# Ignaciagothe/tda-eeg-audio

Hardware: AMD Instinct MI355X
Metric: windows/sec end-to-end (dist->Rips H0/H1->Wasserstein), 47-ch EEG (higher is better)
Workload: dtype f64; 1 GPU; configs[4]+configs[2]: 1416 recordings x 5 bands x 15 selected windows = 106200 (EEG 47x250 f64, audio 250 f64) window pairs per pass, the whole job; per pair corr->dist->Rips H0/H1 (EEG 47 pts), tau per recording-band, Takens dim 3 sub 2 + Rips (audio, 23..123 pts over the bands), Wasserstein H0+H1, features, per-recording reductions; one all-gather of the (1416, 5x48) rows per pass; windows_per_pass=106200, windows_per_gpu_per_pass=106200, input_bytes_per_gpu=10195200000, batches_per_pass=1, windows_per_batch=106200, parallelism=recordings dealt over 1 rank(s), one all-gather per pass, batches_in_flight=3, hip_graph=True, batches_rerun_with_full_ladder=0

## Files before the change

### tda_eeg_audio_amd/csrc/corr_dist_dev.h

```cpp
#pragma once
#include "common.h"

#ifndef CD_TCH
#define CD_TCH 32
#define CD_TSH 5
#endif
#define CD_MAXCH 64

typedef double d4 __attribute__((ext_vector_type(4)));



template <int NPRE>
__device__ __forceinline__ void cd_fetch(double (&pre)[NPRE], const double* __restrict__ X, int ld, int n_ch, int c0,
                                         int tc, int tid)
{
    constexpr int CPK = 256 / CD_TCH;
    const int t = tid & (CD_TCH - 1), ch0 = tid >> CD_TSH;
    const int toff = ch0 * ld + t;
    const bool live = t < tc;
#pragma unroll
    for (int k = 0; k < NPRE; ++k) {
        const double* rowk = X + (size_t)(CPK * k) * (size_t)ld + c0;
        pre[k] = (live && ch0 + CPK * k < n_ch) ? rowk[toff] : 0.0;
    }
}
template <int NPRE, int CSP>
__device__ __forceinline__ void cd_stash(const double (&pre)[NPRE], double* tile, const double* mean, int n_ch, int tc,
                                         int tid, bool centre)
{
    double m[NPRE];
#pragma unroll
    for (int k = 0; k < NPRE; ++k) m[k] = centre ? mean[(tid + 256 * k) >> CD_TSH] : 0.0;
    const int t = tid & (CD_TCH - 1);
    const bool live = t < tc;
#pragma unroll
    for (int k = 0; k < NPRE; ++k) {
        const int ch = (tid + 256 * k) >> CD_TSH;
        tile[t * CSP + ch] = live ? pre[k] - m[k] : 0.0;
    }
}

#define CD_RES_CHUNKS (256 / CD_TCH)


template <int NB>
struct CdLayout {
    static constexpr int CP = 16 * NB;
    static constexpr int CSP = CP + 1;
    static constexpr int NBLK = NB * (NB + 1) / 2;
    static constexpr int TILE = CD_TCH * CSP;
    static constexpr int ACCS = NBLK * 256;
    static constexpr size_t BYTES = sizeof(double) * ((size_t)TILE + ACCS + 2 * CP);
    __device__ static __forceinline__ int acc_index(int i, int j)
    {
        const int lo = i < j ? i : j, hi = i < j ? j : i;
        const int r = lo >> 4, s = hi >> 4;
        const int b = r * NB - ((r * (r - 1)) >> 1) + (s - r);
        return (b * 4 + ((lo & 15) >> 2)) * 64 + ((lo & 3) << 4) + (hi & 15);
    }
};

template <int NB, bool RES>
__device__ __forceinline__ void cd_window_products(unsigned char* smem, const double* __restrict__ X, int n_ch, int n_t,
                                                   int ld)
{
    constexpr int CP = 16 * NB;
    constexpr int CSP = CP + 1;
    constexpr int NPRE = CP * CD_TCH / 256;
    constexpr int NBLK = NB * (NB + 1) / 2;
    constexpr int MAXQ = (NBLK + 3) / 4;
    constexpr int NBUF = RES ? CD_RES_CHUNKS : 1;
    double* tile = reinterpret_cast<double*>(smem);
    double* accs = tile + CD_TCH * CSP;
    double* mean = accs + NBLK * 256;
    double* sdev = mean + CP;
    const int tid = threadIdx.x, l = tid & 63, wv = uni(tid >> 6);
    const int n_chunks = (n_t + CD_TCH - 1) / CD_TCH;
    double pre[NBUF][NPRE];
    auto chunk_len = [&](int c) { const int r = n_t - c * CD_TCH; return r < CD_TCH ? r : CD_TCH; };
    const double* lane_base = tile + (l >> 4) * CSP + (l & 15);

    d4 sacc = (d4){0.0, 0.0, 0.0, 0.0};
    auto sum_tile = [&](int tc) {
        if (wv < NB) {
            const double* p0 = lane_base + 16 * wv;
            const int ntr = (tc + 15) >> 4;
            double a[2][2];
            a[0][0] = p0[0]; a[0][1] = p0[4 * CSP];
            for (int d = 0; d < ntr; ++d) {
                const double* p1 = p0 + (16 * d + 8) * CSP;
                a[1][0] = p1[0]; a[1][1] = p1[4 * CSP];
                sacc = __builtin_amdgcn_mfma_f64_16x16x4f64(a[0][0], 1.0, sacc, 0, 0, 0);
                sacc = __builtin_amdgcn_mfma_f64_16x16x4f64(a[0][1], 1.0, sacc, 0, 0, 0);
                const double* p2 = p0 + (16 * d + 16 < CD_TCH ? 16 * d + 16 : 0) * CSP;
                a[0][0] = p2[0]; a[0][1] = p2[4 * CSP];
                sacc = __builtin_amdgcn_mfma_f64_16x16x4f64(a[1][0], 1.0, sacc, 0, 0, 0);
                sacc = __builtin_amdgcn_mfma_f64_16x16x4f64(a[1][1], 1.0, sacc, 0, 0, 0);
            }
            }
    };
    if constexpr (RES) {
#pragma unroll
        for (int c = 0; c < NBUF; ++c)
            if (c < n_chunks) cd_fetch<NPRE>(pre[c], X, ld, n_ch, c * CD_TCH, chunk_len(c), tid);
#pragma unroll
        for (int c = 0; c < NBUF; ++c)
            if (c < n_chunks) {
                cd_stash<NPRE, CSP>(pre[c], tile, mean, n_ch, chunk_len(c), tid, false);
                __syncthreads();
                sum_tile(chunk_len(c));
                __syncthreads();
            }
    } else {
        cd_fetch<NPRE>(pre[0], X, ld, n_ch, 0, chunk_len(0), tid);
        for (int c = 0; c < n_chunks; ++c) {
            cd_stash<NPRE, CSP>(pre[0], tile, mean, n_ch, chunk_len(c), tid, false);
            __syncthreads();
            const int c1 = (c + 1 < n_chunks) ? c + 1 : 0;
            cd_fetch<NPRE>(pre[0], X, ld, n_ch, c1 * CD_TCH, chunk_len(c1), tid);
            sum_tile(chunk_len(c));
            __syncthreads();
        }
    }
    if (wv < NB && (l & 15) == 0) {
#pragma unroll
        for (int v = 0; v < 4; ++v) {
            const int ch = 16 * wv + 4 * v + (l >> 4);
            mean[ch] = ch < n_ch ? sacc[v] / (double)n_t : 0.0;
        }
    }
    __syncthreads();

    auto mfma_tile = [&](int c, int tc) {
        int br[MAXQ], bs[MAXQ], bb[MAXQ];
        d4 acc[MAXQ];
        const int b0 = (wv + 4 * NBLK - ((c * NBLK) & 3)) & 3;
#pragma unroll
        for (int q = 0; q < MAXQ; ++q) {
            int b = b0 + 4 * q, r = 0;
            bb[q] = b;
            if (b >= NBLK) b = 0;
            while (b >= NB - r) { b -= NB - r; ++r; }
            br[q] = r; bs[q] = r + b;
            if (bb[q] < NBLK && c > 0) {
#pragma unroll
                for (int v = 0; v < 4; ++v) acc[q][v] = accs[(bb[q] * 4 + v) * 64 + l];
            } else acc[q] = (d4){0.0, 0.0, 0.0, 0.0};
        }
        double oa[2][MAXQ][2], ob[2][MAXQ][2];
        auto load_ops = [&](int trip, int s) {
#pragma unroll
            for (int q = 0; q < MAXQ; ++q)
                if (bb[q] < NBLK) {
#pragma unroll
                    for (int u = 0; u < 2; ++u) {
                        const double* p = lane_base + (8 * trip + 4 * u) * CSP;
                        oa[s][q][u] = p[16 * br[q]];
                        ob[s][q][u] = p[16 * bs[q]];
                    }
                }
        };
        auto run_ops = [&](int s) {
#pragma unroll
            for (int u = 0; u < 2; ++u)
#pragma unroll
                for (int q = 0; q < MAXQ; ++q)
                    if (bb[q] < NBLK) acc[q] = __builtin_amdgcn_mfma_f64_16x16x4f64(oa[s][q][u], ob[s][q][u], acc[q], 0, 0, 0);
        };
        const int ntr = (tc + 15) >> 4;
        load_ops(0, 0);
        for (int d = 0; d < ntr; ++d) {
            load_ops(2 * d + 1, 1);
            run_ops(0);
            load_ops(2 * d + 2 < CD_TCH / 8 ? 2 * d + 2 : 0, 0);
            run_ops(1);
        }
#pragma unroll
        for (int q = 0; q < MAXQ; ++q)
            if (bb[q] < NBLK) {
#pragma unroll
                for (int v = 0; v < 4; ++v) accs[(bb[q] * 4 + v) * 64 + l] = acc[q][v];
            }
    };
    if constexpr (RES) {
#pragma unroll
        for (int c = 0; c < NBUF; ++c)
            if (c < n_chunks) {
                cd_stash<NPRE, CSP>(pre[c], tile, mean, n_ch, chunk_len(c), tid, true);
                __syncthreads();
                mfma_tile(c, chunk_len(c));
                __syncthreads();
            }
    } else {
        for (int c = 0; c < n_chunks; ++c) {
            cd_stash<NPRE, CSP>(pre[0], tile, mean, n_ch, chunk_len(c), tid, true);
            __syncthreads();
            if (c + 1 < n_chunks) cd_fetch<NPRE>(pre[0], X, ld, n_ch, (c + 1) * CD_TCH, chunk_len(c + 1), tid);
            mfma_tile(c, chunk_len(c));
            __syncthreads();
        }
    }

    const double fact = 1.0 / (double)(n_t - 1);
    if (tid < n_ch) sdev[tid] = sqrt(accs[CdLayout<NB>::acc_index(tid, tid)] * fact);
    __syncthreads();
}
```

### tda_eeg_audio_amd/csrc/rips.hip

```cpp
#include "common.h"
#include "corr_dist_dev.h"
#include "rips_ladder.h"
#include "rips_keys_dev.h"
#include <stdlib.h>

static_assert(TDA_RETRY_AUTO == rips_ladder::AUTO && TDA_RETRY_FIRST_PASS == rips_ladder::FIRST_PASS &&
              TDA_RETRY_ONLY == rips_ladder::ONLY && TDA_RETRY_ONE_STEP == rips_ladder::ONE_STEP &&
              TDA_RETRY_LAST_RUNG == rips_ladder::LAST_RUNG, "rips_ladder::plan takes tda_ctx::retry_policy as it is");

#ifndef CLOUD_NB
#define CLOUD_NB 8192
#endif
#ifndef NARROW_NT
#define NARROW_NT 512
#endif
#ifndef NARROW_WAVES
#define NARROW_WAVES 6
#endif
#if defined(TDA_PROFILE) && !defined(TDA_PROFILE_STOPS_ONLY)
#define NARROW_NB (NARROW_NT == 384 ? 1536 : 1024)
#else
#define NARROW_NB (NARROW_NT == 384 ? 1536 : 2048)
#endif
#define NARROW_EMAX 7626
#define NT_MAX 512
#define RANK_NONE 0x7fffu

#ifdef TDA_PROFILE
__device__ unsigned long long g_prof[48];
#ifdef TDA_PROFILE_STOPS_ONLY
#define PROF_BEGIN() do {} while (0)
#define PROF_RESUME() do {} while (0)
#define PROF_MARK(i) do {} while (0)
#define PROF_COUNT(i, v) do {} while (0)
#define PROF_FLUSH() do {} while (0)
#else
__shared__ unsigned long long prof_lds[48];
#define PROF_BEGIN()                                                       \
    if (threadIdx.x < 48) prof_lds[threadIdx.x] = 0ull;                    \
    __syncthreads();                                                       \
    unsigned long long prof_t0 = clock64()
#define PROF_RESUME() unsigned long long prof_t0 = clock64()
#define PROF_MARK(i)                                                       \
    do {                                                                   \
        unsigned long long prof_t1 = clock64();                            \
        if (threadIdx.x == 0) prof_lds[i] += prof_t1 - prof_t0;            \
        prof_t0 = prof_t1;                                                 \
    } while (0)
#define PROF_COUNT(i, v) do { if (threadIdx.x == 0) prof_lds[i] += (unsigned long long)(v); } while (0)
#define PROF_FLUSH()                                                       \
    do {                                                                   \
        __syncthreads();                                                   \
        if (threadIdx.x < 48 && prof_lds[threadIdx.x]) atomicAdd(&g_prof[threadIdx.x], prof_lds[threadIdx.x]); \
    } while (0)
#endif
__device__ int g_stop_after;
extern "C" __attribute__((visibility("default"))) int tda_profile_stop_after(int n)
{
    return hipMemcpyToSymbol(HIP_SYMBOL(g_stop_after), &n, sizeof(int)) != hipSuccess;
}
#define PROF_STOP(n, cleanup) do { if (g_stop_after == (n)) { cleanup; return; } } while (0)
#define PROF_STOPC(n, cleanup) do { if (g_stop_after == (n) + 100 * prof_chunk) { cleanup; return; } } while (0)
extern "C" __attribute__((visibility("default"))) int tda_profile_read(unsigned long long* out, int reset)
{
    if (hipMemcpyFromSymbol(out, HIP_SYMBOL(g_prof), sizeof(unsigned long long) * 48) != hipSuccess) return 1;
    if (reset) {
        unsigned long long z[48] = {0};
        if (hipMemcpyToSymbol(HIP_SYMBOL(g_prof), z, sizeof(z)) != hipSuccess) return 1;
    }
    return 0;
}
#else
#define PROF_BEGIN() do {} while (0)
#define PROF_RESUME() do {} while (0)
#define PROF_MARK(i) do {} while (0)
#define PROF_COUNT(i, v) do {} while (0)
#define PROF_FLUSH() do {} while (0)
#define PROF_STOP(n, cleanup) do {} while (0)
#define PROF_STOPC(n, cleanup) do {} while (0)
#endif

#define LDS_ORDER() asm volatile("" ::: "memory")

#define LAUNDER(v) asm volatile("" : "+v"(v))
#define WAVE_SYNC()                                            \
    do {                                                       \
        __builtin_amdgcn_fence(__ATOMIC_ACQ_REL, "workgroup"); \
        __builtin_amdgcn_wave_barrier();                       \
    } while (0)

struct SweepShared {
    u64 alive[8];
    int cov_min[2], status, spare, k1, nk, more;
};

typedef unsigned short pk_u16 __attribute__((ext_vector_type(2)));
typedef short pk_i16 __attribute__((ext_vector_type(2)));

template <int W, typename WT>
struct __attribute__((aligned(sizeof(WT)))) Psi {
    WT w[W];
};
template <int W, typename WT>
__device__ __forceinline__ Psi<W, WT> pxor(Psi<W, WT> a, Psi<W, WT> b)
{
    Psi<W, WT> r;
#pragma unroll
    for (int i = 0; i < W; ++i) r.w[i] = a.w[i] ^ b.w[i];
    return r;
}
template <int W, typename WT>
__device__ __forceinline__ bool pnz(Psi<W, WT> a)
{
    WT o = 0;
#pragma unroll
    for (int i = 0; i < W; ++i) o |= a.w[i];
    return o != 0;
}
template <int W, typename WT>
__device__ __forceinline__ Psi<W, WT> pzero()
{
    Psi<W, WT> r;
#pragma unroll
    for (int i = 0; i < W; ++i) r.w[i] = 0;
    return r;
}

__device__ __forceinline__ double wave_min_f64(double v)
{
#pragma unroll
    for (int off = 32; off > 0; off >>= 1) { const double o = __shfl_xor(v, off, 64); v = o < v ? o : v; }
    return v;
}
__device__ __forceinline__ double wave_max_f64(double v)
{
#pragma unroll
    for (int off = 32; off > 0; off >>= 1) { const double o = __shfl_xor(v, off, 64); v = o > v ? o : v; }
    return v;
}

#ifndef TDA_NO_EDGE_TABLE
struct EdgeTable {
    u16 v[8192 + 512];
    constexpr EdgeTable() : v()
    {
        int a = 1, b = 0;
        for (int e = 0; e < 8192 + 512; ++e) { v[e] = (u16)((a << 8) | b); if (++b == a) { ++a; b = 0; } }
    }
};
__device__ const EdgeTable g_edge_ab = EdgeTable();
__device__ __forceinline__ u32 edge_ab(int e) { return (u32)g_edge_ab.v[e]; }
#else
__device__ __forceinline__ u32 edge_ab(int e) { const int a = edge_row(e); return (u32)((a << 8) | (e - tri2(a))); }
#endif

struct WgVote {
    u32* slots;
    int parity;
};
template <int NT>
__device__ __forceinline__ bool wg_any(WgVote& v, bool p)
{
    static_assert(NT % 64 == 0 && NT <= 512, "slots are read as one or two 16-byte words; slots beyond NT / 64 hold zero");
    const bool w = __ballot(p) != 0ull;
    u32* s = v.slots + 8 * v.parity;
    if ((threadIdx.x & 63) == 0) s[threadIdx.x >> 6] = w ? 1u : 0u;
    __syncthreads();
    v.parity ^= 1;
    const uint4 x = *reinterpret_cast<const uint4*>(s);
    u32 r = x.x | x.y | x.z | x.w;
    if (NT > 256) { const uint4 y = *reinterpret_cast<const uint4*>(s + 4); r |= y.x | y.y | y.z | y.w; }
    return r != 0u;
}
template <int NT>
__device__ __forceinline__ bool wg_all(WgVote& v, bool p) { return !wg_any<NT>(v, !p); }

__device__ __forceinline__ int wave_incl_scan_i32(int v)
{
#define TDA_DPP_ADD_(CTRL, RM) v += __builtin_amdgcn_update_dpp(0, v, CTRL, RM, 0xF, true)
    TDA_DPP_ADD_(0x111, 0xF);
    TDA_DPP_ADD_(0x112, 0xF);
    TDA_DPP_ADD_(0x114, 0xF);
    TDA_DPP_ADD_(0x118, 0xF);
    TDA_DPP_ADD_(0x142, 0xA);
    TDA_DPP_ADD_(0x143, 0xC);
#undef TDA_DPP_ADD_
    return v;
}

__device__ __forceinline__ u32 wave_shr1_u32(u32 v) { return (u32)__builtin_amdgcn_update_dpp(0, (int)v, 0x138, 0xF, 0xF, true); }

template <int W, typename WT>
__device__ __forceinline__ Psi<W, WT> last_nonzero_of_owner(Psi<W, WT> y, u32 own1)
{
    constexpr int H = (int)sizeof(WT) / 4;
    u32 x[W * H];
    {
        const bool mine = wave_shr1_u32(own1) == own1;
#pragma unroll
        for (int i = 0; i < W * H; ++i) {
            const u32 below = wave_shr1_u32((u32)((u64)y.w[i / H] >> (32 * (i % H))));
            x[i] = mine ? below : 0u;
        }
    }
#define TDA_STEP_(CTRL)                                                                                              \
    {                                                                                                                \
        u32 any = 0u;                                                                                                \
        _Pragma("unroll") for (int i = 0; i < W * H; ++i) any |= x[i];                                               \
        const bool take = any == 0u && (u32)__builtin_amdgcn_update_dpp(0, (int)own1, CTRL, 0xF, 0xF, true) == own1; \
        _Pragma("unroll") for (int i = 0; i < W * H; ++i) {                                                          \
            const u32 o = (u32)__builtin_amdgcn_update_dpp(0, (int)x[i], CTRL, 0xF, 0xF, true);                      \
            x[i] = take ? o : x[i];                                                                                  \
        }                                                                                                            \
    }
    TDA_STEP_(0x111) TDA_STEP_(0x112) TDA_STEP_(0x114)
#undef TDA_STEP_
    Psi<W, WT> r;
#pragma unroll
    for (int c = 0; c < W; ++c) {
        if constexpr (H == 2) r.w[c] = (WT)(((u64)x[2 * c + 1] << 32) | x[2 * c]);
        else r.w[c] = (WT)x[c];
    }
    return r;
}

__device__ __forceinline__ int edge_flat(u32 pk) { return tri2((int)(pk >> 8)) + (int)(pk & 255u); }

struct Bucketer {
    float dmin, scale, top;
    __device__ __forceinline__ int operator()(u32 key) const
    {
        const float x = fminf((sortable_f32(key) - dmin) * scale, top);
        const int b = (int)x;
        return b < 0 ? 0 : b;
    }
};

template <int NT>
__device__ __forceinline__ void effective_threshold(int n, u32 tkey, const u32* vmax, u32 kmin_thread, u32* red, u32& teff_out, u32& kmin_out)
{
    const int tid = threadIdx.x;
    const int lane = tid & 63;
    const u32 m0 = lane < n ? vmax[lane] : 0xffffffffu, m1 = lane + 64 < n ? vmax[lane + 64] : 0xffffffffu;
    const u32 renc = wave_min_u32_dpp(m0 < m1 ? m0 : m1);
    teff_out = renc < tkey ? renc : tkey;
    if (tid == 0) red[1] = 0xffffffffu;
    __syncthreads();
    const u32 kmin = wave_min_u32_dpp(kmin_thread);
    if (lane == 63) atomicMin(&red[1], kmin);
    __syncthreads();
    kmin_out = red[1];
}

template <int NT, int NB, bool WANT_KEYS>
__device__ __forceinline__ int rank_edges(const u32* key32, int E, u32 teff, u32 kmin, u16* members, u32* cursor, int* wsum, u16* rank,
                          u16* ord, u32* skey)
{
    static_assert(NB % (2 * NT) == 0, "every thread scans whole words");
    constexpr int WPT = NB / NT / 2;
    const int tid = threadIdx.x, lane = tid & 63, wave = tid >> 6;
    Bucketer bk;
    bk.dmin = sortable_f32(kmin);
    bk.top = (float)(NB - 1);
    bk.scale = bk.top / (sortable_f32(teff) - bk.dmin);
    for (int i = tid; i < NB / 2; i += NT) cursor[i] = 0u;
    __syncthreads();
#pragma unroll 4
    for (int e = tid; e < E; e += NT) {
        const u32 k = key32[e];
        u32 b = 0xffffu;
        if (k <= teff) { b = (u32)bk(k); atomicAdd(&cursor[b >> 1], 1u << (16 * (b & 1))); }
        rank[e] = (u16)b;
    }
    __syncthreads();
    {
        u32 w[WPT];
        int s = 0;
#pragma unroll
        for (int i = 0; i < WPT; ++i) {
            const u32 x = cursor[tid * WPT + i];
            const int c0 = (int)(x & 0xffffu), c1 = (int)(x >> 16);
            w[i] = (u32)s | ((u32)(s + c0) << 16);
            s += c0 + c1;
        }
        const int incl = wave_incl_scan_i32(s);
        if (lane == 63) wsum[wave] = incl;
        __syncthreads();
        int basep = incl - s;
        for (int q = 0; q < wave; ++q) basep += wsum[q];
        const u32 add = (u32)basep * 0x00010001u;
#pragma unroll
        for (int i = 0; i < WPT; ++i) cursor[tid * WPT + i] = w[i] + add;
    }
    __syncthreads();
#pragma unroll 4
    for (int e = tid; e < E; e += NT) {
        const u32 b = rank[e];
        if (b != 0xffffu) {
            const int sh = 16 * (int)(b & 1u);
            const u32 old = atomicAdd(&cursor[b >> 1], 1u << sh);
            members[(old >> sh) & 0xffffu] = (u16)e;
        }
    }
    __syncthreads();
    const u16* cur16 = reinterpret_cast<const u16*>(cursor);
    const int Ev = uni((int)cur16[NB - 1]);
#pragma unroll 4
    for (int e = tid; e < E; e += NT) {
        const u32 b = rank[e];
        u32 r = RANK_NONE;
        if (b != 0xffffu) {
            const u32 k = key32[e];
            const int lo = b ? (int)cur16[b - 1] : 0, hi = (int)cur16[b];
            int c = 0;
            for (int j = lo; j < hi; ++j) {
                const u32 m = members[j];
                const u32 km = key32[m];
                c += (km < k || (km == k && m < (u32)e)) ? 1 : 0;
            }
            r = (u32)(lo + c);
        }
        rank[e] = (u16)r;
    }
    __syncthreads();
#pragma unroll 4
    for (int e = tid; e < E; e += NT) {
        const u32 r = rank[e];
        if (r != RANK_NONE) {
            ord[r] = (u16)edge_ab(e);
            if (WANT_KEYS) skey[r] = key32[e];
        }
    }
    __syncthreads();
    return Ev;
}

#if defined(TDA_PROFILE) && !defined(TDA_PROFILE_STOPS_ONLY)
#define NARROW_LDS ((160 * 1024 / 3 / 1280) * 1280 - 384)
#else
#define NARROW_LDS ((160 * 1024 / 3 / 1280) * 1280)
#endif
#define NARROW_PMAX 124
#define NARROW_DIM 3
#ifdef TDA_DEBUG_PTS
#define NL_GUARD 16
#else
#define NL_GUARD 0
#endif
#define NL_A16(x) (((x) + 15) & ~15)
struct NL {
    static constexpr int E = NARROW_EMAX;
    static constexpr int RANK = 0;
    static constexpr int PSI = NL_A16(2 * E) + NL_GUARD;
    static constexpr int MEMBERS = NL_A16(4 * (E + 4));
    static constexpr int CURSOR = NL_A16(MEMBERS + 2 * E);
    static constexpr int RSCR = CURSOR + 2 * NARROW_NB;
    static constexpr int TOTAL = NARROW_LDS;
    static constexpr int AUX = TOTAL - NL_GUARD - NL_A16(NARROW_PMAX * NARROW_DIM * 8);
    static constexpr int MISC = AUX - NL_GUARD - NL_A16(8752 + 8 * 32);
    static constexpr int REGION = MISC - NL_GUARD - PSI;
    static_assert(RSCR + 720 <= AUX - NL_GUARD, "the ranking arrays must end in front of the points");
    static_assert(MEMBERS >= 4 * (E + 4) && CURSOR >= MEMBERS + 2 * E, "room for the walk's padding: skey[E .. E + 3] (rank_edges_narrow)");
    static_assert(E < 0x8000 && RANK_NONE >= E, "rank and flat index of a slot share a register (rank_edges_narrow)");
    static_assert(REGION >= 2 * E + 8 * 512, "the first chunks must fit: class vectors of 2 NT ranks next to the whole of ord");
};

template <int NT, int NB>
__device__ __forceinline__ int rank_edges_narrow(u32* skey, int E, u32 teff, u32 kmin, u16* sidx, u32* cursor, int* wsum,
                                                 u16* rank, u16* ord)
{
    static_assert(NB % (2 * NT) == 0, "every thread scans whole words");
    constexpr int WPT = NB / NT / 2;
    constexpr int EPT = (NARROW_EMAX + NT - 1) / NT;
    static_assert(EPT <= 32, "one bit per edge of the thread");
    const int tid = threadIdx.x, lane = tid & 63, wave = tid >> 6;
    Bucketer bk;
    bk.dmin = sortable_f32(kmin);
    bk.top = (float)(NB - 1);
    bk.scale = bk.top / (sortable_f32(teff) - bk.dmin);
    for (int i = tid; i < NB / 2; i += NT) cursor[i] = 0u;
    __syncthreads();
    u32 kreg[EPT], breg[EPT];
    u32 beyond = 0u;
#pragma unroll
    for (int i = 0; i < EPT; ++i) {
        const int e = tid + i * NT;
        breg[i] = 0xffffffffu;
        if (e < E) {
            const u32 k = skey[e];
            kreg[i] = k;
            if (k <= teff) { const u32 b = (u32)bk(k); breg[i] = b; atomicAdd(&cursor[b >> 1], 1u << (16 * (b & 1))); }
            else beyond |= 1u << i;
        }
    }
    __syncthreads();
    {
        u32 w[WPT];
        int s = 0;
#pragma unroll
        for (int i = 0; i < WPT; ++i) {
            const u32 x = cursor[tid * WPT + i];
            const int c0 = (int)(x & 0xffffu), c1 = (int)(x >> 16);
            w[i] = (u32)s | ((u32)(s + c0) << 16);
            s += c0 + c1;
        }
        const int incl = wave_incl_scan_i32(s);
        if (lane == 63) wsum[wave] = incl;
        __syncthreads();
        int basep = incl - s;
        for (int q = 0; q < wave; ++q) basep += wsum[q];
        const u32 add = (u32)basep * 0x00010001u;
#pragma unroll
        for (int i = 0; i < WPT; ++i) cursor[tid * WPT + i] = w[i] + add;
        if (tid == NT - 1) {
            const int total = basep + s;
            skey[total] = 0xffffffffu; skey[total + 1] = 0xffffffffu; skey[total + 2] = 0xffffffffu; skey[total + 3] = 0xffffffffu;
        }
    }
    __syncthreads();
#pragma unroll
    for (int i = 0; i < EPT; ++i) {
        const u32 b = breg[i];
        if (b != 0xffffffffu) {
            const int sh = 16 * (int)(b & 1u);
            const u32 slot = (atomicAdd(&cursor[b >> 1], 1u << sh) >> sh) & 0xffffu;
            skey[slot] = kreg[i];
            sidx[slot] = (u16)(tid + i * NT);
        }
    }
    __syncthreads();
    const u16* cur16 = reinterpret_cast<const u16*>(cursor);
    const int Ev = uni((int)cur16[NB - 1]);
    u32 re[EPT];
#pragma unroll
    for (int i = 0; i < EPT; ++i) {
        const int s = tid + i * NT;
        re[i] = 0xffffffffu;
        if (s < Ev) {
            const u32 k = skey[s];
            const u32 e = (u32)sidx[s];
            const u32 b = (u32)bk(k);
            const int lo = b ? (int)cur16[b - 1] : 0, hi = (int)cur16[b];
            int c = 0;
            u32 q = 4u * (u32)lo;
            const u32 q_hi = 4u * (u32)hi, q_end = 4u * (u32)Ev;
            u64 once = 0ull, twice = 0ull;
#pragma unroll 1
            do {
                const u32* p = reinterpret_cast<const u32*>(reinterpret_cast<const unsigned char*>(skey) + min(q, q_end));
                u32 km[4];
#pragma unroll
                for (int t = 0; t < 4; ++t) km[t] = p[t];
#pragma unroll
                for (int t = 0; t < 4; ++t) {
                    c += km[t] < k ? 1 : 0;
                    const u64 m = __ballot(km[t] == k);
                    twice |= once & m;
                    once |= m;
                }
                q += 16u;
            } while (__any(q < q_hi));
            if ((twice >> lane) & 1ull) {
                c = 0;
#pragma unroll 1
                for (int j = lo; j < hi; ++j) {
                    const u32 km = skey[j];
                    c += (km < k || (km == k && (u32)sidx[j] < e)) ? 1 : 0;
                }
            }
            re[i] = ((u32)(lo + c) << 16) | e;
        }
    }
    __syncthreads();
#pragma unroll
    for (int i = 0; i < EPT; ++i) {
        if (re[i] != 0xffffffffu) {
            const u32 r = re[i] >> 16, e = re[i] & 0xffffu;
            rank[e] = (u16)r;
            ord[r] = (u16)edge_ab((int)e);
        }
        if (beyond & (1u << i)) rank[tid + i * NT] = (u16)RANK_NONE;
    }
    __syncthreads();
    return Ev;
}

struct RipsOut {
    double* h0; int h0_cap; int* h0_cnt;
    double* h1; int h1_cap; int* h1_cnt;
    int* status;
    int* retry_list = nullptr;
};

struct RipsLayout {
    int off_members;
    int off_rank, off_ord, off_aux, off_misc;
    int total;
    int off_psi, psi_bytes, off_cursor, off_rscr;
    int guard[5], n_guard;
};

#define TDA_WIN_LDS_GUARD 0x100
#ifndef TDA_SOLO_PRIO
#define TDA_SOLO_PRIO 3
#endif
#define TDA_SOLO_BEGIN() __builtin_amdgcn_s_setprio(TDA_SOLO_PRIO)
#define TDA_SOLO_END() __builtin_amdgcn_s_setprio(0)

#define TDA_POLL_LIMIT (1 << 16)
#ifndef TDA_TURN_SLEEP
#define TDA_TURN_SLEEP 4
#endif
#ifdef TDA_DEBUG_PTS
__device__ int g_fault;
extern "C" __attribute__((visibility("default"))) int tda_debug_inject(int what)
{
    return hipMemcpyToSymbol(HIP_SYMBOL(g_fault), &what, sizeof(int)) != hipSuccess;
}
#define TDA_FAULT(n) (g_fault == (n))
#else
#define TDA_FAULT(n) false
#endif
#ifdef TDA_DEBUG_PTS
#define GUARD_BYTES 16
__device__ __forceinline__ void guard_write(unsigned char* smem, const RipsLayout& L)
{
    if ((int)threadIdx.x < 4 * L.n_guard) reinterpret_cast<u32*>(smem + L.guard[threadIdx.x >> 2] - GUARD_BYTES)[threadIdx.x & 3] = 0xC0FFEE00u + threadIdx.x;
    __syncthreads();
}
__device__ __forceinline__ int guard_check(unsigned char* smem, const RipsLayout& L)
{
    __syncthreads();
    bool bad = false;
    if ((int)threadIdx.x < 4 * L.n_guard) bad = reinterpret_cast<u32*>(smem + L.guard[threadIdx.x >> 2] - GUARD_BYTES)[threadIdx.x & 3] != 0xC0FFEE00u + threadIdx.x;
    return __syncthreads_or(bad ? 1 : 0) ? TDA_WIN_LDS_GUARD : 0;
}
#else
#define GUARD_BYTES 0
__device__ __forceinline__ void guard_write(unsigned char*, const RipsLayout&) {}
__device__ __forceinline__ int guard_check(unsigned char*, const RipsLayout&) { return 0; }
#endif

#define MISC_COMP 0
#define MISC_CAND 512
#define MISC_WV (512 + 128)
#define MISC_MIN (512 + 192)
#define MISC_DONE (512 + 208)
#define MISC_SORTCNT (512 + 224)
#define MISC_SHARED (MISC_DONE + NT_MAX)
#define MISC_CKEY (MISC_SHARED + 96)
#define MISC_LIST MISC_CKEY
#define MISC_LIST_BYTES (4 * NT_MAX + 1280)
#define MISC_ADJ (MISC_LIST + MISC_LIST_BYTES)
#define MISC_ADJC (MISC_ADJ + 128 * 16)
#define MISC_BRANK (MISC_ADJC + 128 * 16)
#define MISC_BYTES(ncls) (MISC_BRANK + 8 * (ncls))

template <int NT, int NVW, int W, typename WT, bool NARROW, class KEYFN>
__device__ __forceinline__ void rips_sweep(int n, int E, int Ev, const u16* rank, const u16* ord, Psi<W, WT>* psi, int psi_bytes,
                           unsigned char* misc, KEYFN keyfn, double* h0, int h0_cap, double* h1, int h1_cap,
                           int& out_k0, int& out_k1, int& out_status)
{
    static_assert(!NARROW || W == 1, "the narrow layout is the point-cloud first pass");
    int psi_cap = 0;
    const int tid0 = threadIdx.x;
    const int lane0 = tid0 & 63, wave = uni(tid0 >> 6);
    int* brank = reinterpret_cast<int*>(misc + MISC_BRANK);
    u64* cand = reinterpret_cast<u64*>(misc + MISC_CAND);
    unsigned char* done = misc + MISC_DONE;
    SweepShared* shared = reinterpret_cast<SweepShared*>(misc + MISC_SHARED);
    u64* adj = reinterpret_cast<u64*>(misc + MISC_ADJ);
    constexpr int WB = 8 * (int)sizeof(WT);
    float* bkey = reinterpret_cast<float*>(misc + MISC_BRANK + 4 * WB * W);
    u64* adjc = reinterpret_cast<u64*>(misc + MISC_ADJC);
    int* tcum = reinterpret_cast<int*>(misc + MISC_COMP + 256);
    int* ecum = reinterpret_cast<int*>(misc + MISC_COMP + 320);
    int eset = 0;

    if constexpr (!NARROW) for (int e = tid0; e < E; e += NT) psi[e] = pzero<W, WT>();
    for (int i = tid0; i < WB * W; i += NT) { brank[i] = -1; bkey[i] = 0.f; }
    for (int i = tid0; i < 256; i += NT) { adj[i] = 0ull; adjc[i] = 0ull; }
    if (tid0 == 0) {
        u32* lc = reinterpret_cast<u32*>(misc + MISC_MIN);
        lc[0] = 0u; lc[1] = 0xffffffffu; lc[2] = 0u;
        lc[3] = 0u;
        shared->status = 0;
    }
    if (tid0 < 16) {
        reinterpret_cast<u32*>(misc + MISC_WV)[tid0] = 0u;
        cand[tid0] = 0ull;
    }
    __syncthreads();

    WgVote vote{reinterpret_cast<u32*>(misc + MISC_WV), 0};
    WT alive[W];
#pragma unroll
    for (int c = 0; c < W; ++c) alive[c] = 0;
    int k0 = 0, k1 = 0, merges = 0, status = 0;
    int compA = lane0, compB = lane0 + 64;

    int clen = NT;
    int ordcls = 0;
    int cov_next = tid0;
#ifdef TDA_PROFILE
    int prof_rneed = 0, prof_chunk = -1;
#endif
    PROF_RESUME();
    for (int r0 = 0; r0 < Ev && !status; r0 += clen) {
        int tid = tid0;
        LAUNDER(tid);
        const int lane = tid & 63;
        clen = NT;
        PROF_MARK(15);
#ifdef TDA_PROFILE
        ++prof_chunk;
#endif
        PROF_COUNT(23, 1);
        const int r = r0 + tid;
        const bool valid = r < Ev;
        int a = 1, b = 0;
        if (valid) { const u32 pk = ord[r]; a = (int)(pk >> 8); b = (int)(pk & 255u); }
        const int tab = tri2(a) + b;
        const int slot = NARROW ? r : tab;
        if constexpr (NARROW) {
            psi_cap = (psi_bytes - 2 * (E - r0)) >> 2;
            if (r < psi_cap) psi[r] = pzero<W, WT>();
        }
        u64 M[NVW], M0[NVW];
        u64 Aj[NVW], Bj[NVW];
#pragma unroll
        for (int w = 0; w < NVW; ++w) { M[w] = 0; M0[w] = 0; Aj[w] = 0; Bj[w] = 0; }
        if (valid) {
#pragma unroll
            for (int w = 0; w < NVW; ++w) { Aj[w] = adj[2 * a + w]; Bj[w] = adj[2 * b + w]; M0[w] = Aj[w] & Bj[w]; }
        }
        {
            volatile u32* turn = reinterpret_cast<volatile u32*>(misc + MISC_MIN) + 2;
            if (wave > 0) {
                int trips = 0;
                for (;;) {
                    const u32 t = (u32)uni((int)*turn);
                    if (t >= (u32)wave) break;
                    if (++trips > TDA_POLL_LIMIT) { if (lane == 0) turn[1] = 1u; break; }
                    if (t + 1u < (u32)wave) __builtin_amdgcn_s_sleep(TDA_TURN_SLEEP); else __builtin_amdgcn_s_sleep(0);
                }
            }
            __builtin_amdgcn_fence(__ATOMIC_ACQUIRE, "workgroup");
            if (valid) {
#pragma unroll
                for (int w = 0; w < NVW; ++w) M[w] = (Aj[w] | adjc[2 * a + w]) & (Bj[w] | adjc[2 * b + w]);
                atomicOr(reinterpret_cast<unsigned long long*>(&adjc[2 * a + (b >> 6)]), 1ull << (b & 63));
                atomicOr(reinterpret_cast<unsigned long long*>(&adjc[2 * b + (a >> 6)]), 1ull << (a & 63));
            }
            LDS_ORDER();
            if (lane == 0 && !(TDA_FAULT(1) && wave == 3)) *turn = (u32)wave + 1u;
        }
        if (valid) {
            const int ta0 = tri2(a), tb0 = tri2(b);
#pragma unroll
            for (int w = 0; w < NVW; ++w) {
                u64 cc = (Aj[w] | adjc[2 * a + w]) & (Bj[w] | adjc[2 * b + w]) & ~M[w];
                while (cc) {
                    const int v0 = 64 * w + __builtin_ctzll(cc); cc &= cc - 1ull;
                    const bool ok1 = cc != 0ull; const int v1 = ok1 ? 64 * w + __builtin_ctzll(cc) : v0; cc &= cc - 1ull;
                    const int t0 = tri2(v0), t1 = tri2(v1);
                    const u32 xa0 = rank[v0 < a ? ta0 + v0 : t0 + a], xb0 = rank[v0 < b ? tb0 + v0 : t0 + b];
                    const u32 xa1 = rank[v1 < a ? ta0 + v1 : t1 + a], xb1 = rank[v1 < b ? tb0 + v1 : t1 + b];
                    if ((int)(xa0 > xb0 ? xa0 : xb0) < r) M[w] |= 1ull << (v0 & 63);
                    if (ok1 && (int)(xa1 > xb1 ? xa1 : xb1) < r) M[w] |= 1ull << (v1 & 63);
                }
            }
        }
        u64 many = 0;
#pragma unroll
        for (int w = 0; w < NVW; ++w) many |= M[w];
        const bool is_cand = valid && many == 0;
        int vstar = 0, d1 = 0, d2 = 0, q1 = 0, q2 = 0;
        {
            u64 many0 = 0;
#pragma unroll
            for (int w = 0; w < NVW; ++w) many0 |= M0[w];
            if (many0) {
                if (NVW == 1 || M0[0]) vstar = __builtin_ctzll(M0[0]);
                else vstar = 64 + __builtin_ctzll(M0[NVW - 1]);
            } else if (many) {
                if (NVW == 1 || M[0]) vstar = __builtin_ctzll(M[0]);
                else vstar = 64 + __builtin_ctzll(M[NVW - 1]);
            }
            if (valid && many != 0) {
                d1 = pair_index(a, vstar); d2 = pair_index(b, vstar);
                q1 = (int)rank[d1] - r0; q2 = (int)rank[d2] - r0;
                if (TDA_FAULT(2) && tid == 77 && q1 >= 0) q1 = tid;
            }
        }
        PROF_MARK(4);
        PROF_STOPC(11, out_k0 = k0; out_k1 = k1; out_status = 0);
        u64* mbal = reinterpret_cast<u64*>(misc + MISC_COMP);
        u64* zbal = mbal + 8;
        int* offs = reinterpret_cast<int*>(mbal + 16);
        u16* freebits = reinterpret_cast<u16*>(misc + MISC_CKEY);
        float mykey = 0.f;
        if (is_cand) mykey = keyfn(r, a, b);
        {
            const u64 bal = __ballot(is_cand), zb = __ballot(is_cand && mykey == 0.0f);
            if (lane == 0) { cand[wave] = bal; zbal[wave] = zb; }
        }
        done[tid] = 0;
        if (tid < 9) tcum[tid] = 0;
        __syncthreads();
        PROF_MARK(21);
        PROF_STOPC(12, out_k0 = k0; out_k1 = k1; out_status = 0);
        int nfree = 0;
#pragma unroll
        for (int c = 0; c < W; ++c) nfree += __builtin_popcountll((u64)(WT)~alive[c]);
        int ncand = 0;
#pragma unroll
        for (int w = 0; w < NT / 64; ++w) ncand += __builtin_popcountll(cand[w]);
        int btot = 0;
        if (ncand > 0) {
        const bool par = ncand > 24;
        const int lblA0 = compA, lblB0 = compB;
        int qpar = NT;
        if (par) {
            int* bcomp = reinterpret_cast<int*>(misc + MISC_LIST + 1024);
            u32* bbest2 = reinterpret_cast<u32*>(bcomp + 128);
            int* bpar = reinterpret_cast<int*>(bcomp + 384);
            auto rounds = [&](int limit) {
                if (wave == 0) { bcomp[lane] = lblA0; bcomp[64 + lane] = lblB0; }
                if (tid < 256) bbest2[tid] = 0xffffffffu;
                __syncthreads();
                bool live = is_cand && tid < limit, picked = false;
                for (int round = 0; round < 64; ++round) {
                    u32* bbest = bbest2 + 128 * (round & 1);
                    int ca = 0, cb2 = 0;
                    if (live) {
                        ca = bcomp[a]; cb2 = bcomp[b];
                        if (ca == cb2) live = false;
                        else { atomicMin(&bbest[ca], (u32)tid); atomicMin(&bbest[cb2], (u32)tid); }
                    }
                    if (!wg_any<NT>(vote, live)) break;
                    if (live && (bbest[ca] == (u32)tid || bbest[cb2] == (u32)tid)) { picked = true; live = false; }
                    if (wave == 0) {
                        TDA_SOLO_BEGIN();
                        int pp[2];
#pragma unroll
                        for (int h = 0; h < 2; ++h) {
                            const int me = lane + 64 * h;
                            pp[h] = me;
                            const u32 bp = bbest[me];
                            if (bp != 0xffffffffu) {
                                const u32 pk = ord[r0 + (int)bp];
                                const int oa = bcomp[pk >> 8], ob = bcomp[pk & 255u];
                                pp[h] = oa == me ? ob : oa;
                                if (bbest[pp[h]] == bp && me < pp[h]) pp[h] = me;
                            }
                        }
                        bpar[lane] = pp[0]; bpar[64 + lane] = pp[1];
                        for (int it = 0; it < 8; ++it) {
                            const int p0 = bpar[lane], p1 = bpar[64 + lane];
                            const int g0 = bpar[p0], g1 = bpar[p1];
                            if (__ballot(g0 != p0 || g1 != p1) == 0ull) break;
                            bpar[lane] = g0; bpar[64 + lane] = g1;
                        }
                        const int c0 = bcomp[lane], c1 = bcomp[64 + lane];
                        const int n0 = bpar[c0], n1 = bpar[c1];
                        bcomp[lane] = n0; bcomp[64 + lane] = n1;
                        u32* other = bbest2 + 128 * ((round + 1) & 1);
                        other[lane] = 0xffffffffu; other[64 + lane] = 0xffffffffu;
                        TDA_SOLO_END();
                    }
                    __syncthreads();
                }
                const u64 mb = __ballot(picked);
                if (lane == 0) mbal[wave] = mb;
                __syncthreads();
            };
            rounds(NT);
            int nbirth = 0, wcut = -1, before = 0;
#pragma unroll
            for (int w = 0; w < NT / 64; ++w) {
                const int nb = __builtin_popcountll(cand[w] & ~mbal[w]);
                if (wcut < 0 && nbirth + nb > nfree) { wcut = w; before = nbirth; }
                nbirth += nb;
            }
            if (wcut >= 0) {
                u64 bw = cand[wcut] & ~mbal[wcut];
                for (int k = before; k < nfree; ++k) bw &= bw - 1ull;
                qpar = 64 * wcut + __builtin_ctzll(bw);
                PROF_COUNT(26, 1);
                __syncthreads();
                rounds(qpar);
            }
            if (wave == 0) { compA = bcomp[lane]; compB = bcomp[64 + lane]; }
        }
        if (wave == 0) {
            TDA_SOLO_BEGIN();
            const u64 candv = cand[lane & 7];
            int q = par ? qpar : NT, births = 0;
            const bool walk = !par;
            for (int g = 0; g < NT / 64 && walk; ++g) {
                u64 cb = q == NT ? rl64(candv, g) : 0ull;
                u64 mm = 0ull;
                if (cb) {
                    PROF_COUNT(20, __builtin_popcountll(cb));
                    const u32 pkv = ord[r0 + 64 * g + lane < E ? r0 + 64 * g + lane : E - 1];
                    while (cb) {
                        const int l = __builtin_ctzll(cb);
                        cb &= cb - 1;
                        const u32 pk = rl32(pkv, l);
                        const int qa = (int)(pk >> 8), qb = (int)(pk & 255u);
                        int ca, cbb;
                        if (NVW == 1) {
                            ca = (int)rl32((u32)compA, qa);
                            cbb = (int)rl32((u32)compA, qb);
                        } else {
                            const int a0 = (int)rl32((u32)compA, qa & 63), a1 = (int)rl32((u32)compB, qa & 63);
                            const int b0 = (int)rl32((u32)compA, qb & 63), b1 = (int)rl32((u32)compB, qb & 63);
                            ca = qa < 64 ? a0 : a1;
                            cbb = qb < 64 ? b0 : b1;
                        }
                        const bool same = ca == cbb, open = q == NT;
                        q = (open && same && births == nfree) ? 64 * g + l : q;
                        births += same ? 1 : 0;
                        const int cnew = (q == NT) ? ca : cbb;
                        compA = compA == cbb ? cnew : compA;
                        if (NVW == 2) compB = compB == cbb ? cnew : compB;
                        mm |= (!same && q == NT) ? (1ull << l) : 0ull;
                    }
                }
                if (lane == 0) mbal[g] = mm;
            }
            int nb = 0, nr = 0, nm = 0;
            if (lane < NT / 64) {
                u64 cg = cand[lane];
                if (64 * lane >= q) cg = 0ull;
                else if (q < 64 * lane + 64) cg &= (1ull << (q - 64 * lane)) - 1ull;
                const u64 mg = mbal[lane], zg = zbal[lane];
                nb = __builtin_popcountll(cg & ~mg); nr = __builtin_popcountll(mg & ~zg); nm = __builtin_popcountll(mg);
            }
            int pb = 0, pr = 0, tb = 0, tr = 0, tm = 0;
#pragma unroll
            for (int w = 0; w < NT / 64; ++w) {
                const int xb = (int)rl32((u32)nb, w), xr = (int)rl32((u32)nr, w), xm = (int)rl32((u32)nm, w);
                if (w < lane) { pb += xb; pr += xr; }
                tb += xb; tr += xr; tm += xm;
            }
            if (lane < NT / 64) { offs[lane] = pb; offs[8 + lane] = pr; }
            if (lane == 0) { offs[16] = tb; offs[17] = tr; offs[18] = tm; offs[19] = q; }
            TDA_SOLO_END();
        } else {
            for (int t = tid - 64; t < WB * W; t += NT - 64) {
                const int cw = t / WB, bit = t & (WB - 1);
                int rk = 0;
                bool fr = false;
#pragma unroll
                for (int c = 0; c < W; ++c) {
                    const WT f_ = (WT)~alive[c];
                    if (c < cw) rk += __builtin_popcountll((u64)f_);
                    if (c == cw) { rk += __builtin_popcountll((u64)(f_ & (((WT)1 << bit) - (WT)1))); fr = (f_ >> bit) & (WT)1; }
                }
                if (fr) freebits[rk] = (u16)t;
            }
        }
        __syncthreads();
        PROF_MARK(22);
        PROF_STOPC(13, out_k0 = k0; out_k1 = k1; out_status = 0);
        clen = uni(offs[19]);
        if (clen == 0) status |= TDA_WIN_CLASS_OVERFLOW;
        if (clen < NT) PROF_COUNT(14, 1);
        bool mrg = is_cand && ((mbal[wave] >> lane) & 1ull);
        bool birth = is_cand && !mrg && tid < clen;
        bool row = mrg && mykey != 0.0f;
        const u64 below = (1ull << lane) - 1ull;
        const int bpre = offs[wave] + __builtin_popcountll(__ballot(birth) & below);
        const int rpre = offs[8 + wave] + __builtin_popcountll(__ballot(row) & below);
        btot = uni(offs[16]);
        const int rtot = uni(offs[17]), mtot = uni(offs[18]);
        if (!status) {
            if (row) {
                const int pos = k0 + rpre;
                if (pos < h0_cap) { h0[2 * pos] = 0.0; h0[2 * pos + 1] = (double)mykey; }
            }
            k0 += rtot; merges += mtot;
            if (birth) {
                const int idx = (int)freebits[bpre];
                const int cw = idx / WB, bit = idx & (WB - 1);
                Psi<W, WT> nv = pzero<W, WT>();
#pragma unroll
                for (int c = 0; c < W; ++c)
                    if (c == cw) nv.w[c] = ((WT)1 << bit);
                if (!NARROW || r < psi_cap) psi[slot] = nv;
                brank[idx] = r;
                bkey[idx] = mykey;
            }
            if (W == 1 && wave == 0 && btot > 0) {
                const int nal = __builtin_popcountll((u64)alive[0]);
                if (lane >= nal && lane < nal + btot) ordcls = (int)freebits[lane - nal];
            }
            int left = btot;
#pragma unroll
            for (int c = 0; c < W; ++c) {
                const u64 f_ = (u64)(WT)~alive[c];
                const int pc = __builtin_popcountll(f_);
                if (left >= pc) { alive[c] = (WT)~(WT)0; left -= pc; }
                else if (left > 0) {
                    int lo = 0, hi = 63;
                    while (lo < hi) {
                        const int mid = (lo + hi) >> 1;
                        if (__builtin_popcountll(f_ & ((2ull << mid) - 1ull)) >= left) hi = mid; else lo = mid + 1;
                    }
                    alive[c] |= (WT)(f_ & ((2ull << lo) - 1ull));
                    left = 0;
                }
            }
        }
        }
        if (status) break;
        PROF_MARK(5);
        PROF_STOPC(14, out_k0 = k0; out_k1 = k1; out_status = 0);
        bool quiet = btot == 0;
#pragma unroll
        for (int c = 0; c < W; ++c) quiet = quiet && alive[c] == 0;
        u32* lcnt = reinterpret_cast<u32*>(misc + MISC_MIN);
        if (quiet) PROF_COUNT(24, 1);
#ifdef TDA_PROFILE
        if (!quiet) prof_rneed = r0 + clen;
#endif
        if constexpr (NARROW) {
            if (!quiet && r0 + NT > psi_cap) { status |= TDA_WIN_CLASS_OVERFLOW; break; }
        }
        if (!quiet) {
        const bool apparent = valid && many != 0 && tid < clen;
        bool pending = apparent;
        Psi<W, WT> base = pzero<W, WT>();
        const int s1 = NARROW ? q1 + r0 : d1, s2 = NARROW ? q2 + r0 : d2;
        if (apparent && q1 < 0 && q2 < 0) {
            base = pxor(psi[s1], psi[s2]);
            psi[slot] = base;
            pending = false;
        }
        volatile unsigned char* vdone = done;
        LDS_ORDER();
        if (!pending) vdone[tid] = 1;
#ifdef TDA_PROFILE
#ifndef TDA_PROFILE_STOPS_ONLY
        if (pending) atomicAdd(&prof_lds[33], 1ull);
#endif
        PROF_COUNT(34, 1);
#endif
        int idle_trips = 0;
        while (__ballot(pending)) {
            PROF_COUNT(32, 1);
            bool ready = false;
            if (pending) ready = (q1 < 0 || vdone[q1]) && (q2 < 0 || vdone[q2]);
            const u64 rbal = __ballot(ready);
            __builtin_amdgcn_fence(__ATOMIC_ACQUIRE, "workgroup");
            if (ready) {
                base = pxor(psi[s1], psi[s2]);
                psi[slot] = base;
                LDS_ORDER();
                vdone[tid] = 1;
                pending = false;
            }
            if (!rbal) {
                if (++idle_trips > TDA_POLL_LIMIT) {
                    if (lane == 0) reinterpret_cast<volatile u32*>(misc + MISC_MIN)[3] = 1u;
                    if (pending) vdone[tid] = 1;
                    break;
                }
                __builtin_amdgcn_s_sleep(1);
            }
        }
        __syncthreads();
        PROF_MARK(6);
        PROF_STOPC(15, out_k0 = k0; out_k1 = k1; out_status = 0);
        u32 m0, m1, m2 = 0u, m3 = 0u;
        {
            u64 rem[NVW];
#pragma unroll
            for (int w = 0; w < NVW; ++w) rem[w] = 0ull;
            if (apparent) {
                u64 comp[NVW];
#pragma unroll
                for (int w = 0; w < NVW; ++w) comp[w] = 0ull;
                if (NVW == 1 || vstar < 64) comp[0] = 1ull << vstar;
                else comp[NVW - 1] = 1ull << (vstar - 64);
#pragma unroll
                for (int w = 0; w < NVW; ++w) { comp[w] |= adj[2 * vstar + w] & M[w]; rem[w] = M[w] & ~comp[w]; }
                bool changed = true;
                while (changed) {
                    changed = false;
#pragma unroll
                    for (int w = 0; w < NVW; ++w) {
                        u64 rr = rem[w];
                        while (rr) {
                            int u[4]; bool ok[4];
#pragma unroll
                            for (int k = 0; k < 4; ++k) {
                                ok[k] = rr != 0ull;
                                u[k] = ok[k] ? 64 * w + __builtin_ctzll(rr) : vstar;
                                rr &= rr - 1ull;
                            }
                            u64 nb[4][NVW];
#pragma unroll
                            for (int k = 0; k < 4; ++k)
#pragma unroll
                                for (int x = 0; x < NVW; ++x) nb[k][x] = adj[2 * u[k] + x];
#pragma unroll
                            for (int k = 0; k < 4; ++k) {
                                u64 hit = 0ull;
#pragma unroll
                                for (int x = 0; x < NVW; ++x) hit |= nb[k][x] & comp[x];
                                if (ok[k] && hit) {
                                    comp[w] |= 1ull << (u[k] & 63);
                                    rem[w] &= ~(1ull << (u[k] & 63));
                                    changed = true;
                                }
                            }
                        }
                    }
                    u64 anyr = 0ull;
#pragma unroll
                    for (int w = 0; w < NVW; ++w) anyr |= rem[w];
                    if (!anyr) break;
                }
            }
            m0 = (u32)rem[0]; m1 = (u32)(rem[0] >> 32);
            if (NVW == 2) { m2 = (u32)rem[NVW - 1]; m3 = (u32)(rem[NVW - 1] >> 32); }
        }
        PROF_MARK(16);
        PROF_STOPC(16, out_k0 = k0; out_k1 = k1; out_status = 0);
        constexpr int ES = 4 + W * (int)sizeof(WT);
        constexpr bool SORTED = W == 1;
        constexpr int LMAX = SORTED ? MISC_LIST_BYTES / ES : 256;
        constexpr int LCAP = (MISC_LIST_BYTES / ES) < LMAX ? (MISC_LIST_BYTES / ES) : LMAX;
        constexpr int LPL = (LCAP + 63) / 64;
        static_assert(LCAP * ES <= MISC_LIST_BYTES, "the list stays inside its area");
        constexpr bool FTAB = WB * W * (int)sizeof(Psi<W, WT>) <= MISC_LIST_BYTES;
        constexpr int KMAX = FTAB ? 64 : LCAP;
        unsigned char* list = misc + MISC_LIST;
        u32* tlist = reinterpret_cast<u32*>(adjc);
        static_assert(4 * NT <= 128 * 16 && NT / 64 <= 8, "the work list lives in adjc; nine words per sum");
        const bool cum_lane = lane == 8 || (lane < 8 && lane > wave);
        const int ntri = __builtin_popcount(m0) + __builtin_popcount(m1) + __builtin_popcount(m2) + __builtin_popcount(m3);
        int tstart, ttot;
        const int incl_ = wave_incl_scan_i32(ntri);
        const int wtri = __builtin_amdgcn_readlane(incl_, 63);
        {
            if (wtri != 0 && cum_lane) atomicAdd(&tcum[lane], wtri);
            __syncthreads();
            tstart = tcum[wave] + incl_ - ntri;
            ttot = uni(tcum[8]);
        }
#ifdef TDA_PROFILE
        {
            const int ntri = __builtin_popcount(m0) + __builtin_popcount(m1) + __builtin_popcount(m2) + __builtin_popcount(m3);
#ifndef TDA_PROFILE_STOPS_ONLY
            if (ntri) atomicAdd(&prof_lds[27], (unsigned long long)ntri);
            if (apparent) atomicAdd(&prof_lds[28], 1ull);
            if (ntri) atomicAdd(&prof_lds[29], 1ull);
#endif
        }
#endif
        int list_rounds = 0;
        while (true) {
            u64 left[NVW];
            left[0] = (u64)m0 | ((u64)m1 << 32);
            if (NVW == 2) left[NVW - 1] = (u64)m2 | ((u64)m3 << 32);
            int nxt = tstart;
            int lbase = 0;
#ifdef TDA_PROFILE
            {
                PROF_COUNT(43, (ttot + NT - 1) / NT); PROF_COUNT(44, ttot); PROF_COUNT(47, 1);
#ifndef TDA_PROFILE_STOPS_ONLY
                if (wtri != 0 && lane == 0) atomicAdd(&prof_lds[45], 1ull);
#endif
            }
#endif
            for (int t0 = 0; t0 < ttot; t0 += NT) {
                int* ec = ecum + 16 * eset;
                eset ^= 1;
                if (tid < 9) ec[tid] = 0;
#pragma unroll
                for (int wi = 0; wi < NVW; ++wi) {
                    while (left[wi] != 0ull && (u32)(nxt - t0) < (u32)NT) {
                        const int v = 64 * wi + __builtin_ctzll(left[wi]);
                        left[wi] &= left[wi] - 1ull;
                        tlist[nxt - t0] = ((u32)tid << 8) | (u32)v;
                        ++nxt;
                    }
                }
                __syncthreads();
                u32 code = 0u;
                Psi<W, WT> y = pzero<W, WT>();
                bool keep = false;
                u64 kb = 0ull;
                if (t0 + (wave << 6) < ttot) {
                    const bool item = t0 + tid < ttot;
                    if (item) {
                        code = tlist[tid];
                        const int op = (int)(code >> 8), v = (int)(code & 255u);
                        const u32 pk = ord[r0 + op];
                        const int oa = (int)(pk >> 8), ob = (int)(pk & 255u);
                        const int ta_ = tri2(oa), tb_ = tri2(ob);
                        const int tv = (int)(__umul24((u32)v, (u32)(v - 1)) >> 1);
                        const int fa = v < oa ? ta_ + v : tv + oa;
                        const int fb = v < ob ? tb_ + v : tv + ob;
                        const int ja = NARROW ? (int)rank[fa] : fa;
                        const int jb = NARROW ? (int)rank[fb] : fb;
                        y = pxor(pxor(psi[ja], psi[jb]), psi[NARROW ? r0 + op : ta_ + ob]);
                    }
                    const Psi<W, WT> pv = last_nonzero_of_owner(y, item ? (code >> 8) + 1u : 0u);
                    keep = pnz(y) && pnz(pxor(y, pv));
                    kb = __ballot(keep);
                }
                if (kb != 0ull && cum_lane) atomicAdd(&ec[lane], __builtin_popcountll(kb));
                __syncthreads();
                const int pos = lbase + ec[wave] + (int)__builtin_amdgcn_mbcnt_hi((u32)(kb >> 32), __builtin_amdgcn_mbcnt_lo((u32)kb, 0u));
                lbase += uni(ec[8]);
                if (keep && pos < LCAP) {
                    *reinterpret_cast<u32*>(list + ES * pos) = code;
#pragma unroll
                    for (int c = 0; c < W; ++c)
                        *reinterpret_cast<WT*>(list + ES * pos + 4 + c * (int)sizeof(WT)) = y.w[c];
                }
            }
            if (lbase == 0) {
                PROF_MARK(17);
                PROF_STOPC(17, out_k0 = k0; out_k1 = k1; out_status = 0);
                break;
            }
            __syncthreads();
            PROF_MARK(17);
            PROF_STOPC(17, out_k0 = k0; out_k1 = k1; out_status = 0);
            const u32 cnt = (u32)lbase;
            const bool complete = cnt <= (u32)LCAP;
            PROF_COUNT(11, 1);
            PROF_COUNT(12, cnt);
            if (!complete) PROF_COUNT(13, 1);
            if (cnt > 2u * (u32)LCAP) PROF_COUNT(46, 1);
            WT alive_before[W];
#pragma unroll
            for (int c = 0; c < W; ++c) alive_before[c] = alive[c];
            if (wave == 0) {
                TDA_SOLO_BEGIN();
                const int nl = complete ? (int)cnt : LCAP;
                constexpr int LREG = SORTED ? 1 : LPL;
                u32 ek[LREG];
                Psi<W, WT> ev[LREG];
                auto load_block = [&](int q, u32& k, Psi<W, WT>& x) {
                    const int idx = lane + 64 * q;
                    k = 0xffffffffu; x = pzero<W, WT>();
                    if (idx < nl) {
                        k = *reinterpret_cast<const u32*>(list + ES * idx);
#pragma unroll
                        for (int c = 0; c < W; ++c)
                            x.w[c] = *reinterpret_cast<const WT*>(list + ES * idx + 4 + c * (int)sizeof(WT));
                    }
                };
#pragma unroll
                for (int q = 0; q < LREG; ++q) load_block(q, ek[q], ev[q]);
                const int lb = lane & (WB - 1);
                int brk[W];
                float bky[W];
#pragma unroll
                for (int c = 0; c < W; ++c) {
                    brk[c] = lane < WB ? brank[WB * c + lb] : -1;
                    bky[c] = lane < WB ? bkey[WB * c + lb] : 0.f;
                }
                int nalive0 = W == 1 ? __builtin_popcountll((u64)alive[0]) : 0;
                Psi<W, WT> vimg = pzero<W, WT>();
                u32 mycode = 0u, myrk = 0u;
                float mybirth = 0.f;
                int nk = 0, more = 0;
                const int nq = (nl + 63) >> 6;
                PROF_MARK(30);
                if constexpr (SORTED) {
                    WT kvec = 0;
                    WT cm = lane < nalive0 ? (WT)1 << ordcls : (WT)0;
                    bool stop = false;
                    for (int q = 0; q < nq && !stop; ++q) {
                        WT v = ev[0].w[0];
                        const u32 myk = ek[0];
                        if (q + 1 < nq) load_block(q + 1, ek[0], ev[0]);
                        for (int k = 0; k < nk; ++k) {
                            const WT m = (WT)1 << rl32(mycode, k);
                            const WT w = sizeof(WT) == 8 ? (WT)rl64((u64)kvec, k) : (WT)rl32((u32)kvec, k);
                            if (v & m) v ^= w;
                        }
                        u64 nz = __ballot(v != 0);
                        while (nz) {
                            if (nk == KMAX) { more = 1; stop = true; break; }
                            const int src = __builtin_ctzll(nz);
                            const WT wvw = sizeof(WT) == 8 ? (WT)rl64((u64)v, src) : (WT)rl32((u32)v, src);
                            const u64 ob = __ballot((cm & wvw) != 0);
                            if (!ob) { status |= TDA_WIN_CLASS_OVERFLOW; stop = true; break; }
                            const int opos = 63 - __builtin_clzll(ob);
                            const int ybit = (int)rl32((u32)ordcls, opos);
                            const WT ybm = (WT)1 << ybit;
                            if (v & ybm) v ^= wvw;
                            nz = __ballot(v != 0);
                            const u32 kk = rl32(myk, src);
                            const float ybirth = __uint_as_float(rl32(__float_as_uint(bky[0]), ybit));
                            cm &= (WT)~ybm;
                            const bool me = lane == nk;
                            WT vi = vimg.w[0];
                            if (vi & ybm) vi ^= wvw;
                            vimg.w[0] = me ? (WT)(wvw & (WT)~ybm) : vi;
                            mycode = me ? (u32)ybit : mycode;
                            myrk = me ? (u32)(r0 + (int)((kk >> 8) & 0xffffu)) : myrk;
                            mybirth = me ? ybirth : mybirth;
                            kvec = me ? wvw : kvec;
                            alive[0] &= (WT)~ybm;
                            ++nk;
                        }
                    }
                    if (nk > 0) {
                        const bool keep = cm != 0;
                        const u64 keepb = __ballot(keep);
                        const int below = (int)__builtin_amdgcn_mbcnt_hi((u32)(keepb >> 32), __builtin_amdgcn_mbcnt_lo((u32)keepb, 0u));
                        const int dst = keep ? below : __builtin_popcountll(keepb) + (lane - below);
                        ordcls = __builtin_amdgcn_ds_permute(dst << 2, ordcls);
                    }
                } else
                while (true) {
                    u32 mk = 0xffffffffu;
#pragma unroll
                    for (int q = 0; q < LPL; ++q)
                        if (q < nq && pnz(ev[q]) && ek[q] < mk) mk = ek[q];
                    const u32 best = wave_min_u32_dpp(mk);
                    if (best == 0xffffffffu) break;
                    if (nk == KMAX) { more = 1; break; }
                    const int src = __builtin_ctzll(__ballot(mk == best));
                    Psi<W, WT> mine = pzero<W, WT>();
#pragma unroll
                    for (int q = 0; q < LPL; ++q)
                        if (q < nq && ek[q] == best) mine = ev[q];
                    Psi<W, WT> wv;
#pragma unroll
                    for (int c = 0; c < W; ++c) {
                        if (sizeof(WT) == 8) wv.w[c] = (WT)rl64((u64)mine.w[c], src);
                        else wv.w[c] = (WT)rl32((u32)mine.w[c], src);
                    }
                    const int rk = r0 + (int)(best >> 8);
                    int ybit, ycw;
                    float ybirth;
                    if (W == 1) {
                        const u64 ob = __ballot(lane < nalive0 && (((u64)wv.w[0] >> ordcls) & 1ull));
                        if (!ob) { status |= TDA_WIN_CLASS_OVERFLOW; break; }
                        const int opos = 63 - __builtin_clzll(ob);
                        ybit = (int)rl32((u32)ordcls, opos);
                        ycw = 0;
                        ybirth = __uint_as_float(rl32(__float_as_uint(bky[0]), ybit));
                        const int up = __builtin_amdgcn_update_dpp(0, ordcls, 0x130, 0xF, 0xF, true);
                        if (lane >= opos) ordcls = up;
                        --nalive0;
                    } else {
                        int candv = -1, cwl = 0;
                        float byl = 0.f;
#pragma unroll
                        for (int c = 0; c < W; ++c)
                            if (lane < WB && ((wv.w[c] >> lb) & (WT)1) && brk[c] > candv) { candv = brk[c]; cwl = c; byl = bky[c]; }
                        const int bestr = wave_max_i32_dpp(candv);
                        const u64 ybal = __ballot(candv == bestr && candv >= 0);
                        if (!ybal) { status |= TDA_WIN_CLASS_OVERFLOW; break; }
                        ybit = __builtin_ctzll(ybal);
                        ycw = (int)rl32((u32)cwl, ybit);
                        ybirth = __uint_as_float(rl32(__float_as_uint(byl), ybit));
                    }
                    if (FTAB) {
                        WT sel = 0;
#pragma unroll
                        for (int c = 0; c < W; ++c)
                            if (c == ycw) sel = (vimg.w[c] >> ybit) & (WT)1;
                        if (lane < nk && sel) vimg = pxor(vimg, wv);
                        if (lane == nk) {
                            vimg = wv;
#pragma unroll
                            for (int c = 0; c < W; ++c)
                                if (c == ycw) vimg.w[c] &= (WT)~((WT)1 << ybit);
                            mycode = ((u32)ycw << 8) | (u32)ybit; myrk = (u32)rk; mybirth = ybirth;
                        }
                    } else {
                        const u32 pkk = ord[rk];
                        const float key = keyfn(rk, (int)(pkk >> 8), (int)(pkk & 255u));
                        if (key > ybirth) {
                            if (k1 < h1_cap && lane == 0) { h1[2 * k1] = (double)ybirth; h1[2 * k1 + 1] = (double)key; }
                            ++k1;
                        }
                        if (lane == 0) {
                            *reinterpret_cast<u32*>(list + ES * nk) = ((u32)ycw << 8) | (u32)ybit;
#pragma unroll
                            for (int c = 0; c < W; ++c) *reinterpret_cast<WT*>(list + ES * nk + 4 + c * (int)sizeof(WT)) = wv.w[c];
                        }
                    }
#pragma unroll
                    for (int q = 0; q < LPL; ++q) {
                        if (q >= nq) break;
                        WT sel = 0;
#pragma unroll
                        for (int c = 0; c < W; ++c)
                            if (c == ycw) sel = (ev[q].w[c] >> ybit) & (WT)1;
                        if (sel) ev[q] = pxor(ev[q], wv);
                    }
#pragma unroll
                    for (int c = 0; c < W; ++c)
                        if (c == ycw) alive[c] &= (WT)~((WT)1 << ybit);
                    ++nk;
                }
                PROF_MARK(31);
                PROF_COUNT(10, nk);
                if (FTAB) {
                    const bool mine_ok = lane < nk;
                    float key = 0.f;
                    if (mine_ok) {
                        const u32 pkk = ord[(int)myrk];
                        key = keyfn((int)myrk, (int)(pkk >> 8), (int)(pkk & 255u));
                    }
                    const bool emit = mine_ok && key > mybirth;
                    const u64 bal = __ballot(emit);
                    const int pos = k1 + __builtin_popcountll(bal & ((1ull << lane) - 1ull));
                    if (emit && pos < h1_cap) { h1[2 * pos] = (double)mybirth; h1[2 * pos + 1] = (double)key; }
                    k1 += __builtin_popcountll(bal);
                    if (mine_ok) {
                        Psi<W, WT>* ftab = reinterpret_cast<Psi<W, WT>*>(list);
                        ftab[WB * (int)(mycode >> 8) + (int)(mycode & 255u)] = vimg;
                    }
                }
                if (lane == 0) {
#pragma unroll
                    for (int c = 0; c < W; ++c) shared->alive[c] = (u64)alive[c];
                    shared->k1 = k1; shared->nk = nk; shared->more = more; shared->status = status;
                }
                TDA_SOLO_END();
            }
            __syncthreads();
            PROF_MARK(18);
            PROF_STOPC(18, out_k0 = k0; out_k1 = k1; out_status = 0);
            WT kmask[W];
#pragma unroll
            for (int c = 0; c < W; ++c) {
                const WT na = sizeof(WT) == 8 ? (WT)uni64(shared->alive[c]) : (WT)uni((int)(u32)shared->alive[c]);
                kmask[c] = alive_before[c] & (WT)~na; alive[c] = na;
            }
            k1 = uni(shared->k1);
            const int nk = uni(shared->nk);
            const bool more = uni(shared->more) != 0;
            status = uni(shared->status);
            if (status) break;
            if (FTAB) {
                const Psi<W, WT>* ftab = reinterpret_cast<const Psi<W, WT>*>(list);
                const int seen_end = r0 + clen < Ev ? r0 + clen : Ev;
#pragma unroll 4
                for (int rr = tid; rr < seen_end; rr += NT) {
                    const int e = NARROW ? rr : edge_flat(ord[rr]);
                    const Psi<W, WT> p = psi[e];
                    WT anyh = 0;
#pragma unroll
                    for (int c = 0; c < W; ++c) anyh |= p.w[c] & kmask[c];
                    if (!anyh) continue;
                    Psi<W, WT> q;
#pragma unroll
                    for (int c = 0; c < W; ++c) q.w[c] = p.w[c] & (WT)~kmask[c];
#pragma unroll
                    for (int c = 0; c < W; ++c) {
                        u64 hh = (u64)(p.w[c] & kmask[c]);
                        while (hh) {
                            const int bit = __builtin_ctzll(hh);
                            hh &= hh - 1ull;
                            q = pxor(q, ftab[WB * c + bit]);
                        }
                    }
                    psi[e] = q;
                }
            } else {
                for (int j0 = 0; j0 < nk; j0 += 4) {
                    u32 kc[4];
                    Psi<W, WT> kw[4];
#pragma unroll
                    for (int j = 0; j < 4; ++j) {
                        const int jj = j0 + j < nk ? j0 + j : j0;
                        kc[j] = j0 + j < nk ? *reinterpret_cast<const u32*>(list + ES * jj) : 0xffffffffu;
#pragma unroll
                        for (int c = 0; c < W; ++c) kw[j].w[c] = *reinterpret_cast<const WT*>(list + ES * jj + 4 + c * (int)sizeof(WT));
                    }
#pragma unroll 4
                    for (int rr = tid; rr < (r0 + clen < Ev ? r0 + clen : Ev); rr += NT) {
                        const int e = NARROW ? rr : edge_flat(ord[rr]);
                        Psi<W, WT> p = psi[e];
                        bool changed = false;
#pragma unroll
                        for (int j = 0; j < 4; ++j) {
                            if (kc[j] == 0xffffffffu) continue;
                            const int jcw = (int)(kc[j] >> 8), jbit = (int)(kc[j] & 255u);
                            WT sel = 0;
#pragma unroll
                            for (int c = 0; c < W; ++c)
                                if (c == jcw) sel = (p.w[c] >> jbit) & (WT)1;
                            if (sel) { p = pxor(p, kw[j]); changed = true; }
                        }
                        if (changed) psi[e] = p;
                    }
                }
            }
            PROF_MARK(19);
            PROF_STOPC(19, out_k0 = k0; out_k1 = k1; out_status = 0);
            if (complete && !more) break;
            if (++list_rounds > 4 * NT) { status |= TDA_WIN_CLASS_OVERFLOW; break; }
            __syncthreads();
        }
        }
        if (valid && tid < clen) {
            atomicOr(reinterpret_cast<unsigned long long*>(&adj[2 * a + (b >> 6)]), 1ull << (b & 63));
            atomicOr(reinterpret_cast<unsigned long long*>(&adj[2 * b + (a >> 6)]), 1ull << (a & 63));
        }
        if (tid < 256) adjc[tid] = 0ull;
        if (tid == 0) {
            lcnt[0] = 0u; lcnt[1] = 0xffffffffu; lcnt[2] = 0u; shared->cov_min[0] = 0x7fffffff;
            if (lcnt[3]) shared->status = TDA_WIN_NOT_CONVERGED;
        }
        __syncthreads();
        if (uni(shared->status) & TDA_WIN_NOT_CONVERGED) { status |= TDA_WIN_NOT_CONVERGED; break; }
        bool calm = status == 0 && clen == NT;
#pragma unroll
        for (int c = 0; c < W; ++c) calm = calm && alive[c] == 0;
        if (calm && !quiet) PROF_COUNT(2, 1);
        if (calm) {
            int from = r0 + clen;
            int rr = (NT & (NT - 1)) == 0 ? from + ((tid - from) & (NT - 1)) : from + (((tid - from) % NT) + NT) % NT;
            rr = rr > cov_next ? rr : cov_next;
            int ru;
            for (int round = 0;; ++round) {
                PROF_COUNT(41, 1);
                bool covered = true;
                while (rr < Ev) {
                    const u32 pk = ord[rr];
                    const int ea = (int)(pk >> 8), eb = (int)(pk & 255u);
                    u64 common = adj[2 * ea] & adj[2 * eb];
                    if (NVW == 2) common |= adj[2 * ea + 1] & adj[2 * eb + 1];
                    if (common == 0ull) { covered = false; break; }
                    rr += NT;
                }
                int* cmin = &shared->cov_min[round & 1];
                {
                    const u32 wmin = wave_min_u32_dpp(covered ? 0x7fffffffu : (u32)rr);
                    if (lane == 0 && wmin != 0x7fffffffu) atomicMin(reinterpret_cast<unsigned int*>(cmin), wmin);
                }
                __syncthreads();
                ru = uni(*cmin);
                if (ru >= Ev || ru == from) break;
                if (tid == 0) shared->cov_min[(round + 1) & 1] = 0x7fffffff;
                for (int r2 = from + tid; r2 < ru; r2 += NT) {
                    const u32 pk = ord[r2];
                    const int ea = (int)(pk >> 8), eb = (int)(pk & 255u);
                    atomicOr(reinterpret_cast<unsigned long long*>(&adj[2 * ea + (eb >> 6)]), 1ull << (eb & 63));
                    atomicOr(reinterpret_cast<unsigned long long*>(&adj[2 * eb + (ea >> 6)]), 1ull << (ea & 63));
                }
                PROF_COUNT(35, ru - from);
                from = ru;
                __syncthreads();
                if (round == 31) break;
            }
            cov_next = rr;
            if (ru >= Ev) { PROF_COUNT(25, 1); PROF_MARK(7); break; }
            PROF_COUNT(42, 1);
            if (from > r0 + clen) {
                if constexpr (NARROW) {
                    const int cap = (psi_bytes - 2 * (E - from)) >> 2;
                    for (int r2 = r0 + clen + tid; r2 < (from < cap ? from : cap); r2 += NT) psi[r2] = pzero<W, WT>();
                    __syncthreads();
                }
                clen = from - r0;
            }
        }
        PROF_MARK(7);
        PROF_STOPC(20, out_k0 = k0; out_k1 = k1; out_status = 0);
    }
#ifdef TDA_PROFILE
    PROF_COUNT(36, prof_rneed > 4096 ? 1 : 0); PROF_COUNT(37, prof_rneed > 4608 ? 1 : 0); PROF_COUNT(38, prof_rneed > 5120 ? 1 : 0);
    PROF_COUNT(39, prof_rneed); PROF_COUNT(40, Ev);
#endif
    const int ncomp = n - merges;
    for (int i = 0; i < ncomp; ++i) {
        if (k0 < h0_cap && tid0 == 0) { h0[2 * k0] = 0.0; h0[2 * k0 + 1] = (double)INFINITY; }
        ++k0;
    }
#pragma unroll
    for (int c = 0; c < W; ++c) {
        u64 al = (u64)alive[c];
        while (al) {
            const int bit = __builtin_ctzll(al);
            al &= al - 1;
            if (k1 < h1_cap && tid0 == 0) { h1[2 * k1] = (double)bkey[WB * c + bit]; h1[2 * k1 + 1] = (double)INFINITY; }
            ++k1;
        }
    }
    if (k1 > h1_cap) status |= TDA_WIN_H1_TRUNCATED;
    out_k0 = k0; out_k1 = k1; out_status = status;
}


#define TOT_NW 128
#define TOT_SLOTS 8
#define TOT_SLOT_WORDS ((size_t)8128 * TOT_NW)
#define RETRY_GRID 512
#define RETRY_GRID_WIDE 64

template <int NT, class KEYFN>
__device__ __forceinline__ void rips_sweep_total(int n, int E, int Ev, const u16* rank, const u16* ord, float* bkey, unsigned char* misc,
                                 u64* __restrict__ psi_g, KEYFN keyfn, double* h0, int h0_cap, double* h1, int h1_cap,
                                 int& out_k0, int& out_k1, int& out_status)
{
    constexpr int NWV = NT / 64;
    const int tid = threadIdx.x, lane = tid & 63, wave = uni(tid >> 6);
    u64* adj = reinterpret_cast<u64*>(misc + MISC_ADJ);
    int* comp = reinterpret_cast<int*>(misc + MISC_COMP);
    u32* flags = reinterpret_cast<u32*>(misc + MISC_WV);
    u64* yv = reinterpret_cast<u64*>(misc + MISC_LIST);
    u64* cur = yv + TOT_NW;
    u32* nzbit = reinterpret_cast<u32*>(misc + MISC_ADJ + 4096);
    u32* alivebit = nzbit + 256;
    static_assert(MISC_LIST_BYTES >= 2 * TOT_NW * 8, "scratch of the total sweep");
    for (int i = tid; i < 256; i += NT) { adj[i] = 0ull; nzbit[i] = 0u; alivebit[i] = 0u; }
    for (int v = tid; v < 128; v += NT) comp[v] = v;
    __syncthreads();
    int k0 = 0, k1 = 0, merges = 0, nborn = 0, nalive = 0;
    auto stored = [&](int rr) { return (nzbit[rr >> 5] >> (rr & 31)) & 1u; };
    for (int r = 0; r < Ev; ++r) {
        const u32 pk = (u32)uni((int)ord[r]);
        const int a = (int)(pk >> 8), b = (int)(pk & 255u);
        const u64 M0 = uni64(adj[2 * a] & adj[2 * b]), M1 = uni64(adj[2 * a + 1] & adj[2 * b + 1]);
        if ((M0 | M1) == 0ull) {
            const int ca = uni(comp[a]), cb = uni(comp[b]);
            const float key = keyfn(r, a, b);
            __syncthreads();
            if (ca != cb) {
                for (int v = tid; v < n; v += NT) if (comp[v] == cb) comp[v] = ca;
                if (key != 0.0f) {
                    if (tid == 0 && k0 < h0_cap) { h0[2 * k0] = 0.0; h0[2 * k0 + 1] = (double)key; }
                    ++k0;
                }
                ++merges;
            } else {
                const int c = nborn++;
                if (tid == 0) { bkey[c] = key; nzbit[r >> 5] |= 1u << (r & 31); alivebit[c >> 5] |= 1u << (c & 31); }
                for (int w = tid; w < TOT_NW; w += NT) psi_g[(size_t)r * TOT_NW + w] = (w == (c >> 6)) ? 1ull << (c & 63) : 0ull;
                ++nalive;
            }
        } else if (nalive > 0) {
            const int vstar = M0 ? __builtin_ctzll(M0) : 64 + __builtin_ctzll(M1);
            const int s1 = uni((int)rank[pair_index(a, vstar)]), s2 = uni((int)rank[pair_index(b, vstar)]);
            const bool z1 = !stored(s1), z2 = !stored(s2);
            u64 bw = 0ull;
            if (tid < TOT_NW) {
                bw = (z1 ? 0ull : psi_g[(size_t)s1 * TOT_NW + tid]) ^ (z2 ? 0ull : psi_g[(size_t)s2 * TOT_NW + tid]);
                cur[tid] = bw;
            }
            if (lane == 0) flags[wave] = 0u;
            __syncthreads();
            if (__ballot(bw != 0ull) != 0ull && lane == 0) flags[wave] = 1u;
            __syncthreads();
            bool nzr = false;
#pragma unroll
            for (int w = 0; w < NWV; ++w) nzr = nzr || flags[w] != 0u;
            if (nzr) {
                if (tid < TOT_NW) psi_g[(size_t)r * TOT_NW + tid] = bw;
                if (tid == 0) nzbit[r >> 5] |= 1u << (r & 31);
            }
            u64 R0 = M0, R1 = M1;
            if (vstar < 64) R0 &= ~(1ull << vstar); else R1 &= ~(1ull << (vstar - 64));
            float keyr = 0.f;
            bool have_key = false;
            while ((R0 | R1) != 0ull && nalive > 0) {
                __syncthreads();
                int v = -1;
                {
                    u64 t0 = R0, t1 = R1;
                    for (int k = 0; k < wave && (t0 | t1); ++k) { if (t0) t0 &= t0 - 1ull; else t1 &= t1 - 1ull; }
                    if (t0) v = __builtin_ctzll(t0); else if (t1) v = 64 + __builtin_ctzll(t1);
                }
                u64 y0 = 0ull, y1 = 0ull;
                if (v >= 0) {
                    const int ja = uni((int)rank[pair_index(a, v)]), jb = uni((int)rank[pair_index(b, v)]);
                    y0 = cur[lane]; y1 = cur[lane + 64];
                    if (stored(ja)) { y0 ^= psi_g[(size_t)ja * TOT_NW + lane]; y1 ^= psi_g[(size_t)ja * TOT_NW + lane + 64]; }
                    if (stored(jb)) { y0 ^= psi_g[(size_t)jb * TOT_NW + lane]; y1 ^= psi_g[(size_t)jb * TOT_NW + lane + 64]; }
                }
                const bool wnz = __ballot((y0 | y1) != 0ull) != 0ull;
                if (lane == 0) flags[wave] = wnz ? 1u : 0u;
                __syncthreads();
                int first = -1;
#pragma unroll
                for (int w = NWV - 1; w >= 0; --w) if (flags[w]) first = w;
                if (first < 0) {
                    for (int k = 0; k < NWV && (R0 | R1); ++k) { if (R0) R0 &= R0 - 1ull; else R1 &= R1 - 1ull; }
                    continue;
                }
                if (wave == first) {
                    yv[lane] = y0; yv[lane + 64] = y1;
                    int m = y1 ? 64 * (lane + 64) + 63 - __builtin_clzll(y1) : (y0 ? 64 * lane + 63 - __builtin_clzll(y0) : -1);
                    m = wave_max_i32_dpp(m);
                    if (lane == 0) flags[8] = (u32)m;
                }
                __syncthreads();
                const int c = (int)flags[8];
                if (!have_key) { keyr = keyfn(r, a, b); have_key = true; }
                const float birth = bkey[c];
                if (keyr > birth) {
                    if (tid == 0 && k1 < h1_cap) { h1[2 * k1] = (double)birth; h1[2 * k1 + 1] = (double)keyr; }
                    ++k1;
                }
                if (tid == 0) alivebit[c >> 5] &= ~(1u << (c & 31));
                --nalive;
                for (int rr = wave; rr <= r; rr += NWV) {
                    if (!stored(rr)) continue;
                    const u64 wc = psi_g[(size_t)rr * TOT_NW + (c >> 6)];
                    if (!((wc >> (c & 63)) & 1ull)) continue;
                    psi_g[(size_t)rr * TOT_NW + lane] ^= yv[lane];
                    psi_g[(size_t)rr * TOT_NW + lane + 64] ^= yv[lane + 64];
                }
                __syncthreads();
                if (tid < TOT_NW) cur[tid] = stored(r) ? psi_g[(size_t)r * TOT_NW + tid] : 0ull;
            }
        }
        __syncthreads();
        if (tid == 0) { adj[2 * a + (b >> 6)] |= 1ull << (b & 63); adj[2 * b + (a >> 6)] |= 1ull << (a & 63); }
        __syncthreads();
    }
    int status = 0;
    const int ncomp = n - merges;
    for (int i = 0; i < ncomp; ++i) {
        if (k0 < h0_cap && tid == 0) { h0[2 * k0] = 0.0; h0[2 * k0 + 1] = (double)INFINITY; }
        ++k0;
    }
    for (int c = 0; c < nborn; ++c)
        if ((alivebit[c >> 5] >> (c & 31)) & 1u) {
            if (k1 < h1_cap && tid == 0) { h1[2 * k1] = (double)bkey[c]; h1[2 * k1 + 1] = (double)INFINITY; }
            ++k1;
        }
    if (k1 > h1_cap) status |= TDA_WIN_H1_TRUNCATED;
    out_k0 = k0; out_k1 = k1; out_status = status;
}

struct KeyFromLds {
    const u32* skey;
    __device__ __forceinline__ float operator()(int r, int, int) const { return sortable_f32(skey[r]); }
};

template <int NT, int NVW, int W, typename WT, bool TOTAL = false>
__device__ __forceinline__ void rips_dm_rest(unsigned char* smem, const int win, int n, float thresh, const u32* vmax, u32 kmin_thread,
                             const RipsLayout& L, const RipsOut& out, u64* psi_g = nullptr)
{
    const int tid = threadIdx.x;
    const int E = tri2(n);
    u32* key32 = reinterpret_cast<u32*>(smem);
    u16* members = reinterpret_cast<u16*>(smem + L.off_members);
    Psi<W, WT>* psi = reinterpret_cast<Psi<W, WT>*>(smem);
    u16* rank = reinterpret_cast<u16*>(smem + L.off_rank);
    u16* ord = reinterpret_cast<u16*>(smem + L.off_ord);
    u32* skey = reinterpret_cast<u32*>(smem + L.off_aux);
    unsigned char* misc = smem + L.off_misc;
    u32* red = reinterpret_cast<u32*>(misc + MISC_MIN);
    u32* cursor = reinterpret_cast<u32*>(misc + MISC_SORTCNT);
    int* wsum = reinterpret_cast<int*>(misc + MISC_WV);
    const u32 tkey = f32_sortable(thresh);
    u32 teff, kmin;
    PROF_RESUME();
    effective_threshold<NT>(n, tkey, vmax, kmin_thread, red, teff, kmin);
    PROF_STOP(1, if (tid == 0) { out.h0_cnt[win] = 0; out.h1_cnt[win] = 0; out.status[win] = 0; });
    const int Ev = rank_edges<NT, (NVW == 1 ? 2048 : 8192), true>(key32, E, teff, kmin, members, cursor, wsum, rank, ord, skey);
    PROF_MARK(1);
    PROF_STOP(2, if (tid == 0) { out.h0_cnt[win] = 0; out.h1_cnt[win] = 0; out.status[win] = 0; });
    guard_write(smem, L);
    int k0, k1, st;
    KeyFromLds kf{skey};
    if constexpr (TOTAL)
        rips_sweep_total<NT>(n, E, Ev, rank, ord, reinterpret_cast<float*>(smem), misc, psi_g, kf,
                             out.h0 + (size_t)win * out.h0_cap * 2, out.h0_cap,
                             out.h1 + (size_t)win * out.h1_cap * 2, out.h1_cap, k0, k1, st);
    else
    rips_sweep<NT, NVW, W, WT, false>(n, E, Ev, rank, ord, psi, 0, misc, kf,
                       out.h0 + (size_t)win * out.h0_cap * 2, out.h0_cap,
                       out.h1 + (size_t)win * out.h1_cap * 2, out.h1_cap, k0, k1, st);
    st |= guard_check(smem, L);
    PROF_MARK(3);
    PROF_COUNT(8, 1);
    PROF_COUNT(9, E);
    PROF_FLUSH();
    if (tid == 0) { out.h0_cnt[win] = k0; out.h1_cnt[win] = k1; out.status[win] = st; }
}

template <int NT, int NVW, int W, typename WT, bool TOTAL = false>
__device__ __forceinline__ void rips_dm_window(unsigned char* smem, const int win, const double* __restrict__ dm, int n, float thresh,
                               int symmetrise, const RipsLayout& L, const RipsOut& out, u64* psi_g = nullptr)
{
    const int tid = threadIdx.x;
    const int E = tri2(n);
    u32* key32 = reinterpret_cast<u32*>(smem);
    unsigned char* misc = smem + L.off_misc;
    PROF_BEGIN();
    const double* D = dm + (size_t)win * n * n;
    u32* vmax = reinterpret_cast<u32*>(misc + MISC_COMP);
    if (tid < 128) vmax[tid] = 0u;
    __syncthreads();
    u32 kmin_thread = 0xffffffffu;
    for (int e = tid; e < E; e += NT) {
        const int a = edge_row(e), b = e - tri2(a);
        const u32 sk = f32_sortable(dm_key(D, n, a, b, symmetrise));
        key32[e] = sk;
        kmin_thread = sk < kmin_thread ? sk : kmin_thread;
        atomicMax(&vmax[a], sk);
        atomicMax(&vmax[b], sk);
    }
    __syncthreads();
    PROF_MARK(0);
    rips_dm_rest<NT, NVW, W, WT, TOTAL>(smem, win, n, thresh, vmax, kmin_thread, L, out, psi_g);
}

#ifdef TDA_DEBUG_PTS
__device__ double g_dbg[2048];
extern "C" __attribute__((visibility("default"))) int tda_debug_read(double* out)
{
    return hipMemcpyFromSymbol(out, HIP_SYMBOL(g_dbg), sizeof(double) * 2048) != hipSuccess;
}
#endif
struct KeyFromPts {
    const double* pts;
    int dim;
    __device__ __forceinline__ float operator()(int, int a, int b) const
    {
        double na = 0.0, nb = 0.0, dot = 0.0;
        if (dim == 3) {
            const double* pa = pts + 3 * a;
            const double* pb = pts + 3 * b;
            const double a0 = pa[0], a1 = pa[1], a2 = pa[2], b0 = pb[0], b1 = pb[1], b2 = pb[2];
            na = (a0 * a0 + a1 * a1) + a2 * a2;
            nb = (b0 * b0 + b1 * b1) + b2 * b2;
            dot = fma(a2, b2, fma(a1, b1, a0 * b0));
        } else
        for (int k = 0; k < dim; ++k) {
            const double xa = pts[a * dim + k], xb = pts[b * dim + k];
            na += xa * xa;
            nb += xb * xb;
            dot = (k == 0) ? xa * xb : fma(xa, xb, dot);
        }
        double d2 = -2.0 * dot;
        d2 += na;
        d2 += nb;
        if (!(d2 > 0.0)) d2 = 0.0;
        return (float)sqrt(d2);
    }
};

template <int NT>
__device__ __forceinline__ void row_maxima(const u32* key32, u32* vmax, int P)
{
    constexpr int TPV = NT / 128;
    const int tid = threadIdx.x;
    const int v = tid / TPV, part = tid - v * TPV;
    if (v < P) {
        const int t0 = tri2(v);
        u32 m = 0u;
        for (int b = part; b < v; b += TPV) { const u32 k = key32[t0 + b]; m = k > m ? k : m; }
        if (m) atomicMax(&vmax[v], m);
    }
}

__global__ void __launch_bounds__(256) retry_collect_kernel(const int* __restrict__ status, int n_win, int* __restrict__ list)
{
    const int w = blockIdx.x * 256 + (int)threadIdx.x;
    const bool f = w < n_win && (status[w] & TDA_WIN_CLASS_OVERFLOW);
    const u64 bal = __ballot(f);
    if (bal) {
        const int lane = (int)threadIdx.x & 63, lead = __builtin_ctzll(bal);
        int base = 0;
        if (lane == lead) base = atomicAdd(&list[0], __builtin_popcountll(bal));
        base = __builtin_amdgcn_readlane(base, lead);
        if (f) list[4 + base + __builtin_popcountll(bal & ((1ull << lane) - 1ull))] = w;
    }
}
#define RETRY_SCAN_BEGIN(NT_, out_, n_win_)                                                        \
    {                                                                                              \
        int* rl__ = (out_).retry_list;                                                             \
        const int nl__ = uni(rl__[0]);                                                             \
        for (int j__ = blockIdx.x; j__ < nl__; j__ += gridDim.x) {                                 \
            const int win = uni(rl__[4 + j__]);
#define RETRY_SCAN_END()                                                                           \
            __syncthreads();                                                                       \
        }                                                                                          \
        if (threadIdx.x == 0 && atomicAdd(&rl__[1], 1) == (int)gridDim.x - 1) {                    \
            rl__[0] = 0;                                                                           \
            rl__[1] = 0;                                                                           \
        }                                                                                          \
    }

template <int NT, int NVW, int W, typename WT, bool RETRY>
__global__ void __launch_bounds__(NT, (W <= 2 && !RETRY) ? 4 : 2)
rips_dm_kernel(const double* __restrict__ dm, int n_win, int n, float thresh, int symmetrise, RipsLayout L,
               RipsOut out, unsigned long long* __restrict__ retry_ctr)
{
    extern __shared__ __attribute__((aligned(16))) unsigned char smem[];
    if constexpr (!RETRY) {
        if ((int)blockIdx.x < n_win)
            rips_dm_window<NT, NVW, W, WT>(smem, (int)blockIdx.x, dm, n, thresh, symmetrise, L, out);
    } else {
        RETRY_SCAN_BEGIN(NT, out, n_win)
            if (retry_ctr && threadIdx.x == 0) atomicAdd(retry_ctr, 1ull);
            rips_dm_window<NT, NVW, W, WT>(smem, win, dm, n, thresh, symmetrise, L, out);
        RETRY_SCAN_END()
    }
}

template <int NT, int W, typename WT, bool NARROW, bool TOTAL = false>
__device__ __forceinline__ void rips_cloud_window(unsigned char* smem, const int win, const double* __restrict__ src,
                                  const int* __restrict__ tau_or_npts, int n_t_or_pcap, int dim, int subsample,
                                  int mode, int normalise, float thresh, const RipsLayout& L, int p_max,
                                  int* __restrict__ n_points, const RipsOut& out, u64* psi_g = nullptr)
{
    const int tid = threadIdx.x;
    u32* key32 = reinterpret_cast<u32*>(smem);
    u16* members = reinterpret_cast<u16*>(smem + (NARROW ? NL::MEMBERS : L.off_members));
    Psi<W, WT>* psi = reinterpret_cast<Psi<W, WT>*>(smem + (NARROW ? NL::PSI : 0));
    u16* rank = reinterpret_cast<u16*>(smem + (NARROW ? NL::RANK : L.off_rank));
    u16* ord = reinterpret_cast<u16*>(smem + L.off_ord);
    double* pts = reinterpret_cast<double*>(smem + (NARROW ? NL::AUX : L.off_aux));
    unsigned char* misc = smem + (NARROW ? NL::MISC : L.off_misc);
    unsigned char* rscr = smem + (NARROW ? NL::RSCR : L.off_misc);
    u32* red = reinterpret_cast<u32*>(rscr + MISC_MIN);
    double* mm = reinterpret_cast<double*>(rscr + (NARROW ? MISC_CAND : MISC_CKEY));

    double* h0 = out.h0 + (size_t)win * out.h0_cap * 2;
    double* h1 = out.h1 + (size_t)win * out.h1_cap * 2;

    int P;
    const double* base;
    int tau = 0;
    if (mode == 0) {
        tau = tau_or_npts[win];
        const int nn = n_t_or_pcap - (dim - 1) * tau;
        P = nn > 0 ? (nn + subsample - 1) / subsample : 0;
        base = src + (size_t)win * n_t_or_pcap;
    } else {
        P = tau_or_npts[win];
        base = src + (size_t)win * n_t_or_pcap * dim;
    }
    if (n_points && tid == 0) n_points[win] = P;
    if (P > p_max || (mode == 0 && tau < 1)) {
        if (tid == 0) { out.h0_cnt[win] = 0; out.h1_cnt[win] = 0; out.status[win] = TDA_WIN_TOO_LARGE; }
        return;
    }
    if (P < 3) {
        if (tid == 0) {
            if (out.h0_cap > 0) { h0[0] = 0.0; h0[1] = 0.0; }
            if (out.h1_cap > 0) { h1[0] = 0.0; h1[1] = 0.0; }
            out.h0_cnt[win] = 1; out.h1_cnt[win] = 1;
            out.status[win] = TDA_WIN_DEGENERATE;
        }
        return;
    }
    PROF_BEGIN();
    for (int idx = tid; idx < P * dim; idx += NT) {
        const int i = idx / dim, k = idx - i * dim;
        pts[idx] = (mode == 0) ? base[i * subsample + k * tau] : base[idx];
    }
    __syncthreads();
    if (normalise) {
        if ((tid >> 6) < dim) {
            const int k = tid >> 6, l = tid & 63;
            double mn = INFINITY, mx = -INFINITY;
            for (int i = l; i < P; i += 64) {
                const double v = pts[i * dim + k];
                mn = v < mn ? v : mn;
                mx = v > mx ? v : mx;
            }
            mn = wave_min_f64(mn);
            mx = wave_max_f64(mx);
            if (l == 0) { double rg = mx - mn; if (rg == 0.0) rg = 1.0; mm[2 * k] = mn; mm[2 * k + 1] = rg; }
        }
        __syncthreads();
        for (int idx = tid; idx < P * dim; idx += NT) {
            const int k = idx % dim;
            pts[idx] = (pts[idx] - mm[2 * k]) / mm[2 * k + 1];
        }
        __syncthreads();
    }
#ifdef TDA_DEBUG_PTS
    for (int idx = tid; idx < P * dim; idx += NT) g_dbg[idx] = pts[idx];
#endif
    const int E = tri2(P);
    const u32 tkey = f32_sortable(thresh);
    KeyFromPts kf{pts, dim};
    u32* vmax = reinterpret_cast<u32*>(rscr + MISC_COMP);
    u32* cursor = reinterpret_cast<u32*>(smem + (NARROW ? NL::CURSOR : L.off_cursor));
    int* wsum = reinterpret_cast<int*>(rscr + MISC_WV);
    if (tid < 128) vmax[tid] = 0u;
    double* nrm = reinterpret_cast<double*>(cursor);
    if (tid < P) nrm[tid] = KeyFromPtsTab::norm2(pts + tid * dim, dim);
    __syncthreads();
    const KeyFromPtsTab kft{pts, nrm, dim};
    u32 kmin_thread = 0xffffffffu;
    u32 ab_next = edge_ab(tid);
    for (int e = tid; e < E; e += NT) {
        const u32 ab = ab_next;
        ab_next = edge_ab(e + NT);
        const int a = (int)(ab >> 8), b = (int)(ab & 255u);
        const u32 sk = f32_sortable(kft(0, a, b));
        key32[e] = sk;
        kmin_thread = sk < kmin_thread ? sk : kmin_thread;
        atomicMax(&vmax[b], sk);
    }
    __syncthreads();
    row_maxima<NT>(key32, vmax, P);
    __syncthreads();
    u32 teff, kmin;
    effective_threshold<NT>(P, tkey, vmax, kmin_thread, red, teff, kmin);
    PROF_MARK(0);
    PROF_STOP(1, if (tid == 0) { out.h0_cnt[win] = 0; out.h1_cnt[win] = 0; out.status[win] = 0; });
    int Ev;
    if constexpr (NARROW) {
        ord = reinterpret_cast<u16*>(smem + NL::PSI + NL::REGION) - E;
        Ev = rank_edges_narrow<NT, NARROW_NB>(key32, E, teff, kmin, members, cursor, wsum, rank, ord);
    }
    else Ev = rank_edges<NT, CLOUD_NB, false>(key32, E, teff, kmin, members, cursor, wsum, rank, ord, nullptr);
    PROF_MARK(1);
    PROF_STOP(2, if (tid == 0) { out.h0_cnt[win] = 0; out.h1_cnt[win] = 0; out.status[win] = 0; });
    guard_write(smem, L);
    int k0, k1, st;
    if constexpr (TOTAL)
        rips_sweep_total<NT>(P, E, Ev, rank, ord, reinterpret_cast<float*>(smem), misc, psi_g, kf, h0, out.h0_cap, h1, out.h1_cap, k0, k1, st);
    else if (P <= 64)
        rips_sweep<NT, 1, W, WT, NARROW>(P, E, Ev, rank, ord, psi, NL::REGION, misc, kf, h0, out.h0_cap, h1, out.h1_cap, k0, k1, st);
    else
        rips_sweep<NT, 2, W, WT, NARROW>(P, E, Ev, rank, ord, psi, NL::REGION, misc, kf, h0, out.h0_cap, h1, out.h1_cap, k0, k1, st);
    st |= guard_check(smem, L);
    PROF_MARK(3);
    PROF_COUNT(8, 1);
    PROF_COUNT(9, E);
    PROF_FLUSH();
#ifdef TDA_DEBUG_PTS
    __syncthreads();
    for (int idx = tid; idx < P * dim; idx += NT) g_dbg[1024 + idx] = pts[idx];
#endif
    if (tid == 0) { out.h0_cnt[win] = k0; out.h1_cnt[win] = k1; out.status[win] = st; }
}

#ifndef CLOUD_WAVES
#define CLOUD_WAVES 4
#endif
template <int NT, int W, typename WT, bool RETRY, bool NARROW = false>
__global__ void __launch_bounds__(NT, RETRY ? 2 : (NARROW ? NARROW_WAVES : CLOUD_WAVES))
rips_cloud_kernel(const double* __restrict__ src, const int* __restrict__ tau_or_npts, int n_win,
                  int n_t_or_pcap, int dim, int subsample, int mode, int normalise, float thresh,
                  RipsLayout L, int p_max, int* __restrict__ n_points, RipsOut out,
                  unsigned long long* __restrict__ span, unsigned long long* __restrict__ retry_ctr)
{
    extern __shared__ __attribute__((aligned(16))) unsigned char smem[];
    if (span && blockIdx.x == 0 && threadIdx.x == 0)
        atomicExch(&span[0], wall_clock64());
    if constexpr (!RETRY) {
        if ((int)blockIdx.x < n_win)
            rips_cloud_window<NT, W, WT, NARROW>(smem, (int)blockIdx.x, src, tau_or_npts, n_t_or_pcap, dim, subsample, mode,
                                                 normalise, thresh, L, p_max, n_points, out);
    } else {
        RETRY_SCAN_BEGIN(NT, out, n_win)
            if (retry_ctr && threadIdx.x == 0) atomicAdd(retry_ctr + 1, 1ull);
            rips_cloud_window<NT, W, WT, false>(smem, win, src, tau_or_npts, n_t_or_pcap, dim, subsample, mode, normalise,
                                                thresh, L, p_max, n_points, out);
        RETRY_SCAN_END()
    }
    if (span && threadIdx.x == 0) {
        const unsigned long long now = wall_clock64();
        if (atomicAdd(&span[1], 1ull) == (unsigned long long)gridDim.x - 1ull) {
            const unsigned long long first = atomicAdd(&span[0], 0ull);
            atomicAdd(&span[2], now - first);
            atomicAdd(&span[3], 1ull);
            atomicExch(&span[1], 0ull);
        }
    }
}

template <int NT>
__global__ void __launch_bounds__(NT, 2)
rips_dm_total_kernel(const double* __restrict__ dm, int n_win, int n, float thresh, int symmetrise, RipsLayout L,
                     RipsOut out, u64* __restrict__ scratch, unsigned long long* __restrict__ retry_ctr)
{
    extern __shared__ __attribute__((aligned(16))) unsigned char smem[];
    u64* psi_g = scratch + (size_t)blockIdx.x * TOT_SLOT_WORDS;
    RETRY_SCAN_BEGIN(NT, out, n_win)
        if (retry_ctr && threadIdx.x == 0) atomicAdd(retry_ctr + 2, 1ull);
        rips_dm_window<NT, 2, 1, u32, true>(smem, win, dm, n, thresh, symmetrise, L, out, psi_g);
    RETRY_SCAN_END()
}
template <int NT>
__global__ void __launch_bounds__(NT, 2)
rips_cloud_total_kernel(const double* __restrict__ src, const int* __restrict__ tau_or_npts, int n_win, int n_t_or_pcap,
                        int dim, int subsample, int mode, int normalise, float thresh, RipsLayout L, int p_max,
                        int* __restrict__ n_points, RipsOut out, u64* __restrict__ scratch,
                        unsigned long long* __restrict__ retry_ctr)
{
    extern __shared__ __attribute__((aligned(16))) unsigned char smem[];
    u64* psi_g = scratch + (size_t)blockIdx.x * TOT_SLOT_WORDS;
    RETRY_SCAN_BEGIN(NT, out, n_win)
        if (retry_ctr && threadIdx.x == 0) atomicAdd(retry_ctr + 2, 1ull);
        rips_cloud_window<NT, 1, u32, false, true>(smem, win, src, tau_or_npts, n_t_or_pcap, dim, subsample, mode, normalise,
                                                   thresh, L, p_max, n_points, out, psi_g);
    RETRY_SCAN_END()
}

struct WindowSource {
    const double* base; long long win_stride, group_stride; int ld, wins_per_group; const int* sel;
    __device__ __forceinline__ const double* at(int w) const
    {
        const int g = sel ? sel[w] : w;
        const int r = g / wins_per_group, k = g - r * wins_per_group;
        return base + (size_t)r * (size_t)group_stride + (size_t)k * (size_t)win_stride;
    }
    __device__ __forceinline__ int ld_of(int) const { return ld; }
};
struct RaggedWindowSource {
    const double* base; const long long* start; const long long* ld;
    __device__ __forceinline__ const double* at(int w) const { return base + start[w]; }
    __device__ __forceinline__ int ld_of(int w) const { return (int)ld[w]; }
};

template <int NB, bool RES, int W, typename WT, bool TOTAL = false, class SRC>
__device__ __forceinline__ void eeg_one_window(unsigned char* smem, const SRC& src, int w, int n_ch,
                                               int n_t, float thresh, const RipsLayout& L, const RipsOut& out,
                                               double* __restrict__ dist, double* __restrict__ corr,
                                               u64* __restrict__ psi_g = nullptr)
{
    const int tid = threadIdx.x, l = tid & 63, wv = tid >> 6;
    PROF_BEGIN();
    cd_window_products<NB, RES>(smem, src.at(w), n_ch, n_t, src.ld_of(w));
    const double* accs = reinterpret_cast<const double*>(smem) + CdLayout<NB>::TILE;
    const double* sdev = accs + CdLayout<NB>::ACCS + CdLayout<NB>::CP;
    const double fact = 1.0 / (double)(n_t - 1);
    auto dist_at = [&](int i, int j, double* r_out) {
        double r = (accs[CdLayout<NB>::acc_index(i, j)] * fact / sdev[i]) / sdev[j];
        r = r > 1.0 ? 1.0 : r; r = r < -1.0 ? -1.0 : r; if (r != r) r = 0.0;
        if (r_out) *r_out = r;
        double d = sqrt_rn(2.0 * (1.0 - r));
        if (!(d > 0.0) || i == j) d = 0.0;
        return d;
    };
    const int E = tri2(n_ch);
    u32* key32 = reinterpret_cast<u32*>(smem);
    u32* vmax = reinterpret_cast<u32*>(smem + 4 * ((E + 3) & ~3));
    if (tid < 128) vmax[tid] = 0u;
    __syncthreads();
    u32 kmin_thread = 0xffffffffu;
    for (int e = tid; e < E; e += 256) {
        const int a = edge_row(e), b = e - tri2(a);
        double v = (dist_at(a, b, nullptr) + dist_at(b, a, nullptr)) / 2.0;
        if (v < 0.0) v = 0.0;
        const u32 sk = f32_sortable((float)v);
        key32[e] = sk;
        kmin_thread = sk < kmin_thread ? sk : kmin_thread;
        atomicMax(&vmax[a], sk);
        atomicMax(&vmax[b], sk);
    }
    if (dist) {
        double* Dw = dist + (size_t)w * n_ch * n_ch;
        double* Cw = corr ? corr + (size_t)w * n_ch * n_ch : nullptr;
        for (int i = wv; i < n_ch; i += 4)
            if (l < n_ch) {
                double r;
                const double d = dist_at(i, l, &r);
                Dw[i * n_ch + l] = d;
                if (Cw) Cw[i * n_ch + l] = r;
            }
    }
    __syncthreads();
    PROF_MARK(0);
    rips_dm_rest<256, TOTAL ? 2 : 1, W, WT, TOTAL>(smem, w, n_ch, thresh, vmax, kmin_thread, L, out, psi_g);
}

#ifndef TDA_EEG_WIDE_WAVES
#define TDA_EEG_WIDE_WAVES 2
#endif
template <int NB, bool RES, int W, bool RETRY, typename WT>
#ifndef TDA_EEG_WAVES
#define TDA_EEG_WAVES 6
#endif
__global__ void __launch_bounds__(256, (W > 2 || RETRY) ? TDA_EEG_WIDE_WAVES : (RES ? 3 : TDA_EEG_WAVES))
eeg_window_kernel(WindowSource windows, int n_win, int n_ch, int n_t, float thresh, RipsLayout L, RipsOut out,
                  double* __restrict__ dist, double* __restrict__ corr, unsigned long long* __restrict__ retry_ctr)
{
    extern __shared__ __attribute__((aligned(16))) unsigned char smem[];
    if constexpr (!RETRY) {
        if ((int)blockIdx.x < n_win)
            eeg_one_window<NB, RES, W, WT>(smem, windows, (int)blockIdx.x, n_ch, n_t, thresh, L, out, dist, corr);
    } else {
        RETRY_SCAN_BEGIN(256, out, n_win)
            if (retry_ctr && threadIdx.x == 0) atomicAdd(retry_ctr, 1ull);
            eeg_one_window<NB, RES, W, WT>(smem, windows, win, n_ch, n_t, thresh, L, out, dist, corr);
        RETRY_SCAN_END()
    }
}
template <int NB, bool RES, int W, bool RETRY, typename WT>
__global__ void __launch_bounds__(256, (W > 2 || RETRY) ? TDA_EEG_WIDE_WAVES : (RES ? 3 : TDA_EEG_WAVES))
eeg_window_ragged_kernel(RaggedWindowSource windows, int n_win, int n_ch, int n_t, float thresh, RipsLayout L, RipsOut out,
                         double* __restrict__ dist, double* __restrict__ corr, unsigned long long* __restrict__ retry_ctr)
{
    extern __shared__ __attribute__((aligned(16))) unsigned char smem[];
    if constexpr (!RETRY) {
        if ((int)blockIdx.x < n_win)
            eeg_one_window<NB, RES, W, WT>(smem, windows, (int)blockIdx.x, n_ch, n_t, thresh, L, out, dist, corr);
    } else {
        RETRY_SCAN_BEGIN(256, out, n_win)
            if (retry_ctr && threadIdx.x == 0) atomicAdd(retry_ctr, 1ull);
            eeg_one_window<NB, RES, W, WT>(smem, windows, win, n_ch, n_t, thresh, L, out, dist, corr);
        RETRY_SCAN_END()
    }
}
template <int NB, bool RES, class SRC>
__global__ void __launch_bounds__(256, 2)
eeg_window_total_kernel(SRC windows, int n_win, int n_ch, int n_t, float thresh, RipsLayout L, RipsOut out,
                        double* __restrict__ dist, double* __restrict__ corr, u64* __restrict__ scratch,
                        unsigned long long* __restrict__ retry_ctr)
{
    extern __shared__ __attribute__((aligned(16))) unsigned char smem[];
    u64* psi_g = scratch + (size_t)blockIdx.x * TOT_SLOT_WORDS;
    RETRY_SCAN_BEGIN(256, out, n_win)
        if (retry_ctr && threadIdx.x == 0) atomicAdd(retry_ctr + 2, 1ull);
        eeg_one_window<NB, RES, 1, u32, true>(smem, windows, win, n_ch, n_t, thresh, L, out, dist, corr, psi_g);
    RETRY_SCAN_END()
}
template <int NB, bool RES, int W, bool RETRY, typename WT>
static auto eeg_kernel_of(const WindowSource*) { return eeg_window_kernel<NB, RES, W, RETRY, WT>; }
template <int NB, bool RES, int W, bool RETRY, typename WT>
static auto eeg_kernel_of(const RaggedWindowSource*) { return eeg_window_ragged_kernel<NB, RES, W, RETRY, WT>; }

static inline int align16(int x) { return (x + 15) & ~15; }

tda_status retry_lists_reserve(tda_ctx* ctx, int n_win)
{
    if (n_win <= ctx->retry_cap) return TDA_OK;
    const int cap = (n_win + 1023) & ~1023;
    const size_t one = (size_t)cap + 4;
    for (int i = 0; i < TDA_RETRY_SLOTS; ++i) {
        int* q = nullptr;
        TDA_HIP(ctx, hipMalloc((void**)&q, 3 * one * sizeof(int)));
        for (int l = 0; l < 3; ++l)
            TDA_HIP(ctx, hipMemset(q + l * one, 0, 4 * sizeof(int)));
        if (ctx->retry_buf[i]) ctx->retired.push_back(ctx->retry_buf[i]);
        ctx->retry_buf[i] = q; ctx->fin_list[i] = q + one; ctx->ws_list[i] = q + 2 * one;
    }
    ctx->retry_cap = cap;
    return TDA_OK;
}
static int stream_slot(tda_ctx* ctx, hipStream_t st)
{
    int i = 0;
    while (i < ctx->retry_streams && ctx->retry_stream[i] != st) ++i;
    if (i == ctx->retry_streams) {
        if (i < TDA_RETRY_SLOTS) ctx->retry_stream[ctx->retry_streams++] = st;
        else { i = TDA_RETRY_SLOTS - 1; ++ctx->retry_shared; }
    }
    return i;
}
static tda_status retry_list_take(tda_ctx* ctx, int n_win, RipsOut& out, hipStream_t st)
{
    const tda_status rc = retry_lists_reserve(ctx, n_win);
    if (rc != TDA_OK) return rc;
    out.retry_list = ctx->retry_buf[stream_slot(ctx, st)];
    return TDA_OK;
}
tda_status stream_lists_take(tda_ctx* ctx, int n, hipStream_t st, int* slot)
{
    *slot = -1;
    if (n > ctx->retry_cap) {
        hipStreamCaptureStatus cs = hipStreamCaptureStatusNone;
        if (hipStreamIsCapturing(st, &cs) != hipSuccess) { (void)hipGetLastError(); return TDA_OK; }
        if (cs != hipStreamCaptureStatusNone) return TDA_OK;
        const tda_status rc = retry_lists_reserve(ctx, n);
        if (rc != TDA_OK) return rc;
    }
    *slot = stream_slot(ctx, st);
    return TDA_OK;
}
static tda_status retry_collect(tda_ctx* ctx, const RipsOut& out, int n_win, hipStream_t st)
{
    hipLaunchKernelGGL(retry_collect_kernel, dim3((n_win + 255) / 256), dim3(256), 0, st, out.status, n_win, out.retry_list);
    TDA_HIP(ctx, hipGetLastError());
    return TDA_OK;
}

static RipsLayout make_layout(int n, int psi_bytes_per_edge, int aux_bytes, int NT)
{
    RipsLayout L;
    const int E = n * (n - 1) / 2;
    const int psi_bytes = E * psi_bytes_per_edge;
    L.off_rank = align16(psi_bytes) + GUARD_BYTES;
    L.off_ord = align16(L.off_rank + 2 * E) + GUARD_BYTES;
    L.off_members = psi_bytes_per_edge < 8 ? L.off_ord : 4 * E;
    int after_rank = align16(L.off_ord + 2 * E) + GUARD_BYTES;
    L.off_aux = after_rank;
    L.off_misc = align16(L.off_aux + aux_bytes) + GUARD_BYTES;
    int misc_bytes = MISC_BYTES(8 * psi_bytes_per_edge);
    const int nb = (NT == 256 && n <= 64) ? 2048 : (NT == 512 ? CLOUD_NB : 8192);
    if (misc_bytes < MISC_SORTCNT + 2 * nb) misc_bytes = MISC_SORTCNT + 2 * nb;
    L.total = align16(L.off_misc + misc_bytes) + GUARD_BYTES;
    L.off_psi = 0; L.psi_bytes = 0; L.off_cursor = L.off_misc + MISC_SORTCNT; L.off_rscr = L.off_misc;
    L.guard[0] = L.off_rank; L.guard[1] = L.off_ord; L.guard[2] = L.off_aux; L.guard[3] = L.off_misc; L.guard[4] = L.total;
    L.n_guard = 5;
    return L;
}

static RipsLayout make_narrow_layout(int n, int dim)
{
    static_assert(MISC_BYTES(32) == 8752 + 8 * 32, "NL::MISC assumes this");
    RipsLayout L;
    L.off_rank = NL::RANK; L.off_psi = NL::PSI; L.off_members = NL::MEMBERS; L.off_cursor = NL::CURSOR; L.off_rscr = NL::RSCR;
    L.off_aux = NL::AUX; L.off_misc = NL::MISC; L.psi_bytes = NL::REGION; L.off_ord = 0;
    L.total = (n <= NARROW_PMAX && dim <= NARROW_DIM) ? NL::TOTAL : 0;
    L.guard[0] = NL::PSI; L.guard[1] = NL::MISC; L.guard[2] = NL::AUX; L.guard[3] = NL::TOTAL; L.guard[4] = NL::TOTAL;
    L.n_guard = 4;
    return L;
}

static tda_status order_h1(tda_ctx* ctx, double* h1, int h1_cap, int* h1_cnt, int n_win, hipStream_t st)
{
    if (h1_cap < 2 || ctx->h1_order == TDA_ORDER_DEFERRED) return TDA_OK;
    tda_diagram_set one{h1, h1_cnt, h1_cap, 1, nullptr};
    return launch_diagram_finish(ctx, &one, 1, n_win, st);
}

static const int LDS_MAX = 160 * 1024;
#ifndef CLOUD_NT
#define CLOUD_NT 512
#endif

size_t rips_total_scratch_bytes() { return (size_t)TOT_SLOTS * TOT_SLOT_WORDS * sizeof(u64); }

static RipsLayout total_layout(int n, int aux_bytes, int NT)
{
    RipsLayout L = make_layout(n, 4, aux_bytes, NT);
    int need = align16(L.off_misc + MISC_BRANK + 2048) + GUARD_BYTES;
    const int need_rank = align16(L.off_misc + MISC_SORTCNT + 2 * 8192) + GUARD_BYTES;
    if (need < need_rank) need = need_rank;
    if (L.total < need) { L.total = need; L.guard[4] = L.total; }
    return L;
}

enum RipsPass { PASS_FIRST, PASS_RETRY, PASS_LAST };

static unsigned long long* armed_span(const tda_ctx* ctx, int which) { return ctx->probe[which].armed ? ctx->probe[which].span : nullptr; }

template <class K, class... A>
static tda_status launch_pass(tda_ctx* ctx, K kern, RipsPass pass, int rgrid, int nt, int lds, int probe_id, int n_win,
                              const RipsOut& out, hipStream_t st, A... args)
{
    if (lds > 48 * 1024)
        TDA_HIP(ctx, hipFuncSetAttribute(reinterpret_cast<const void*>(kern), hipFuncAttributeMaxDynamicSharedMemorySize, lds));
    const dim3 grid = pass == PASS_LAST ? dim3(TOT_SLOTS) : dim3(pass == PASS_RETRY && rgrid < n_win ? rgrid : n_win);
    if (pass != PASS_FIRST) { const tda_status rc = retry_collect(ctx, out, n_win, st); if (rc != TDA_OK) return rc; }
    {
        ProbeScope probe(ctx, pass == PASS_FIRST ? probe_id : -1, st);
        hipLaunchKernelGGL(kern, grid, dim3(nt), lds, st, args...);
    }
    TDA_HIP(ctx, hipGetLastError());
    return TDA_OK;
}

template <class STEP, class LAST>
static tda_status run_ladder(tda_ctx* ctx, const rips_ladder::Rungs& rungs, int n_win, RipsOut& out, hipStream_t st,
                             STEP step, LAST last)
{
    tda_status rc = retry_list_take(ctx, n_win, out, st);
    const rips_ladder::Plan plan = rips_ladder::plan(ctx->retry_policy, rungs);
    for (int i = 0; rc == TDA_OK && i < plan.n; ++i) rc = step(plan.step[i].cap, plan.step[i].retry);
    if (rc == TDA_OK && plan.last) rc = last();
    if (rc != TDA_OK) return rc;
    return order_h1(ctx, out.h1, out.h1_cap, out.h1_cnt, n_win, st);
}

static auto dm_kernel(bool one_vertex_word, int W, bool retry)
{
    if (!one_vertex_word)
        return W == 1 ? rips_dm_kernel<256, 2, 1, u64, false>
                      : retry ? rips_dm_kernel<256, 2, 2, u64, true> : rips_dm_kernel<256, 2, 2, u64, false>;
    switch (W) {
    case 1: return rips_dm_kernel<256, 1, 1, u64, false>;
    case 2: return retry ? rips_dm_kernel<256, 1, 2, u64, true> : rips_dm_kernel<256, 1, 2, u64, false>;
    case 4: return retry ? rips_dm_kernel<256, 1, 4, u64, true> : rips_dm_kernel<256, 1, 4, u64, false>;
    default: return rips_dm_kernel<256, 1, 8, u64, true>;
    }
}

tda_status launch_rips_dm(tda_ctx* ctx, const double* dm, int n_win, int n, double thresh, int symmetrise,
                          double* h0, int h0_cap, int* h0_cnt, double* h1, int h1_cap, int* h1_cnt, int* status,
                          hipStream_t st)
{
    if (n_win == 0) return TDA_OK;
    if (n < 1 || n > TDA_MAX_POINTS) TDA_FAIL(ctx, TDA_ERR_UNSUPPORTED, "n must be in [1,128]");
    if (h0_cap < n) TDA_FAIL(ctx, TDA_ERR_INVALID, "h0_cap must be >= n");
    RipsOut out{h0, h0_cap, h0_cnt, h1, h1_cap, h1_cnt, status};
    const float th = (float)thresh;
    const int aux = n * (n - 1) / 2 * 4;
    bool fits[4];
    for (int i = 0; i < 4; ++i) fits[i] = make_layout(n, 8 << i, aux, 256).total <= LDS_MAX;
    return run_ladder(ctx, rips_ladder::dm_rungs(ctx->words_dm, n <= 64, fits), n_win, out, st,
        [&](int W, bool retry) {
            const RipsLayout L = make_layout(n, W * 8, aux, 256);
            const int rgrid = W >= 8 ? RETRY_GRID_WIDE : RETRY_GRID;
            return launch_pass(ctx, dm_kernel(n <= 64, W, retry), retry ? PASS_RETRY : PASS_FIRST, rgrid, 256, L.total,
                               TDA_PROBE_RIPS_DM, n_win, out, st, dm, n_win, n, th, symmetrise, L, out, ctx->retry_ctr);
        },
        [&] {
            const RipsLayout L = total_layout(n, aux, 256);
            return launch_pass(ctx, rips_dm_total_kernel<256>, PASS_LAST, 0, 256, L.total, -1, n_win, out, st,
                               dm, n_win, n, th, symmetrise, L, out, ctx->total_scratch, ctx->retry_ctr);
        });
}

template <bool RES, class SRC>
static auto eeg_kernel(const SRC* src, int bits, bool retry)
{
    switch (bits) {
    case 32: return eeg_kernel_of<3, RES, 1, false, u32>(src);
    case 64: return retry ? eeg_kernel_of<3, RES, 1, true, u64>(src) : eeg_kernel_of<3, RES, 1, false, u64>(src);
    case 128: return retry ? eeg_kernel_of<3, RES, 2, true, u64>(src) : eeg_kernel_of<3, RES, 2, false, u64>(src);
    default: return eeg_kernel_of<3, RES, 8, true, u64>(src);
    }
}

template <bool RES, class SRC>
static tda_status launch_eeg_ladder(tda_ctx* ctx, const SRC& win, int n_win, int n_ch, int n_t, float th, RipsOut& out,
                                    double* dist, double* corr, hipStream_t st)
{
    const int aux = n_ch * (n_ch - 1) / 2 * 4;
    const int cd_bytes = (int)((CdLayout<3>::BYTES + 15) & ~(size_t)15);
    return run_ladder(ctx, rips_ladder::eeg_rungs(ctx->words_dm), n_win, out, st,
        [&](int bits, bool retry) -> tda_status {
            RipsLayout L = make_layout(n_ch, bits / 8, aux, 256);
            if ((size_t)L.total < CdLayout<3>::BYTES) L.total = cd_bytes;
            if (L.total > LDS_MAX) TDA_FAIL(ctx, TDA_ERR_UNSUPPORTED, "window too large for LDS");
            const int rgrid = (bits >> 6) >= 8 ? RETRY_GRID_WIDE : RETRY_GRID;
            return launch_pass(ctx, eeg_kernel<RES>(&win, bits, retry), retry ? PASS_RETRY : PASS_FIRST, rgrid, 256, L.total,
                               TDA_PROBE_RIPS_DM, n_win, out, st, win, n_win, n_ch, n_t, th, L, out, dist, corr, ctx->retry_ctr);
        },
        [&] {
            RipsLayout L = total_layout(n_ch, aux, 256);
            if ((size_t)L.total < CdLayout<3>::BYTES) { L.total = cd_bytes; L.guard[4] = L.total; }
            return launch_pass(ctx, eeg_window_total_kernel<3, RES, SRC>, PASS_LAST, 0, 256, L.total, -1, n_win, out, st,
                               win, n_win, n_ch, n_t, th, L, out, dist, corr, ctx->total_scratch, ctx->retry_ctr);
        });
}

template <class SRC>
static tda_status launch_eeg_source(tda_ctx* ctx, const SRC& src, int n_win, int n_ch, int n_t, double thresh,
                                    double* dist, double* corr, double* h0, int h0_cap, int* h0_cnt, double* h1, int h1_cap,
                                    int* h1_cnt, int* status, hipStream_t st)
{
    if (n_win == 0) return TDA_OK;
    if (n_ch < 33 || n_ch > 48) TDA_FAIL(ctx, TDA_ERR_UNSUPPORTED, "the fused EEG kernel takes 33..48 channels (the reference has 47); use tda_corr_dist_batch + tda_rips_dm_batch otherwise");
    if (n_t < 2 || n_t > CD_RES_CHUNKS * CD_TCH) TDA_FAIL(ctx, TDA_ERR_UNSUPPORTED, "the fused EEG kernel takes windows of 2..256 samples (the reference has 250)");
    if (h0_cap < n_ch) TDA_FAIL(ctx, TDA_ERR_INVALID, "h0_cap must be >= n_ch");
    RipsOut out{h0, h0_cap, h0_cnt, h1, h1_cap, h1_cnt, status};
    static const bool stream_twice = getenv("TDA_EEG_RESIDENT") == nullptr;
    return stream_twice ? launch_eeg_ladder<false>(ctx, src, n_win, n_ch, n_t, (float)thresh, out, dist, corr, st)
                        : launch_eeg_ladder<true>(ctx, src, n_win, n_ch, n_t, (float)thresh, out, dist, corr, st);
}

tda_status launch_eeg_windows(tda_ctx* ctx, const double* win, int n_win, int n_ch, int n_t, double thresh, double* dist,
                              double* corr, double* h0, int h0_cap, int* h0_cnt, double* h1, int h1_cap, int* h1_cnt,
                              int* status, hipStream_t st)
{
    const WindowSource src{win, (long long)n_ch * n_t, 0, n_t, 0x7fffffff, nullptr};
    return launch_eeg_source(ctx, src, n_win, n_ch, n_t, thresh, dist, corr, h0, h0_cap, h0_cnt, h1, h1_cap, h1_cnt, status, st);
}

tda_status launch_eeg_sliding(tda_ctx* ctx, const double* sig, int n_rec, int n_ch, int n_samples, int win_len, int step,
                              const int* sel, int n_sel, double thresh, double* dist, double* corr, double* h0, int h0_cap,
                              int* h0_cnt, double* h1, int h1_cap, int* h1_cnt, int* status, int* n_win_out, hipStream_t st)
{
    if (win_len < 2 || step < 1) TDA_FAIL(ctx, TDA_ERR_INVALID, "win_len must be >= 2 and step >= 1");
    const int per_rec = n_samples >= win_len ? (n_samples - win_len) / step + 1 : 0;
    if (n_win_out) *n_win_out = per_rec;
    if (n_rec <= 0 || per_rec == 0) return TDA_OK;
    if ((long long)n_rec * per_rec > 0x7fffffffLL) TDA_FAIL(ctx, TDA_ERR_UNSUPPORTED, "too many windows in one call");
    const int n_out = sel ? n_sel : n_rec * per_rec;
    const WindowSource src{sig, (long long)step, (long long)n_ch * n_samples, n_samples, per_rec, sel};
    return launch_eeg_source(ctx, src, n_out, n_ch, win_len, thresh, dist, corr, h0, h0_cap, h0_cnt, h1, h1_cap, h1_cnt, status, st);
}

tda_status launch_eeg_ragged(tda_ctx* ctx, const double* sig, const long long* start, const long long* ld, int n_win, int n_ch,
                             int win_len, double thresh, double* dist, double* corr, double* h0, int h0_cap, int* h0_cnt,
                             double* h1, int h1_cap, int* h1_cnt, int* status, hipStream_t st)
{
    if (win_len < 2) TDA_FAIL(ctx, TDA_ERR_INVALID, "win_len must be >= 2");
    const RaggedWindowSource src{sig, start, ld};
    return launch_eeg_source(ctx, src, n_win, n_ch, win_len, thresh, dist, corr, h0, h0_cap, h0_cnt, h1, h1_cap, h1_cnt, status, st);
}

static auto cloud_kernel(int bits, bool retry, bool narrow)
{
    switch (bits) {
    case 32: return narrow ? rips_cloud_kernel<NARROW_NT, 1, u32, false, true> : rips_cloud_kernel<CLOUD_NT, 1, u32, false, false>;
    case 64: return retry ? rips_cloud_kernel<CLOUD_NT, 1, u64, true, false> : rips_cloud_kernel<CLOUD_NT, 1, u64, false, false>;
    default: return rips_cloud_kernel<CLOUD_NT, 2, u64, true, false>;
    }
}

tda_status launch_rips_cloud(tda_ctx* ctx, const double* src, const int* aux, int n_win, int n_t_or_pcap, int dim,
                             int subsample, int mode, int normalise, double thresh, double* h0, int h0_cap,
                             int* h0_cnt, double* h1, int h1_cap, int* h1_cnt, int* n_points, int* status,
                             hipStream_t st)
{
    if (n_win == 0) return TDA_OK;
    if (dim < 1 || dim > TDA_MAX_DIM) TDA_FAIL(ctx, TDA_ERR_UNSUPPORTED, "dim must be in [1,4]");
    if (subsample < 1) subsample = 1;
    int p_max;
    if (mode == 0) {
        const int nn = n_t_or_pcap - (dim - 1);
        p_max = nn > 0 ? (nn + subsample - 1) / subsample : 0;
    } else {
        p_max = n_t_or_pcap;
    }
    if (p_max > TDA_MAX_POINTS) p_max = TDA_MAX_POINTS;
#ifdef TDA_EXPERIMENT
    if (getenv("TDA_EXP_PMAX")) p_max = atoi(getenv("TDA_EXP_PMAX"));
#endif
    if (p_max < 3) p_max = 3;
    if (h0_cap < p_max) TDA_FAIL(ctx, TDA_ERR_INVALID, "h0_cap must be >= max points per cloud");
    RipsOut out{h0, h0_cap, h0_cnt, h1, h1_cap, h1_cnt, status};
    const float th = (float)thresh;
    const int aux_bytes = p_max * dim * 8;
    const bool fits128 = make_layout(p_max, 16, aux_bytes, CLOUD_NT).total <= LDS_MAX;
    static const bool no_narrow = getenv("TDA_CLOUD_WIDE_FIRST") != nullptr;
    const bool narrow_ok = !no_narrow && make_narrow_layout(p_max, dim).total != 0;
    return run_ladder(ctx, rips_ladder::cloud_rungs(ctx->words_cloud, fits128), n_win, out, st,
        [&](int bits, bool retry) -> tda_status {
            const bool narrow = bits == 32 && narrow_ok;
            const RipsLayout L = narrow ? make_narrow_layout(p_max, dim) : make_layout(p_max, bits / 8, aux_bytes, CLOUD_NT);
            if (L.total > LDS_MAX || L.total == 0) TDA_FAIL(ctx, TDA_ERR_UNSUPPORTED, "point cloud too large for LDS");
            const int W = bits == 128 ? 2 : 1;
            const int rgrid = W >= 2 ? RETRY_GRID / 2 : RETRY_GRID;
            return launch_pass(ctx, cloud_kernel(bits, retry, narrow), retry ? PASS_RETRY : PASS_FIRST, rgrid,
                               narrow ? NARROW_NT : CLOUD_NT, L.total, TDA_PROBE_RIPS_CLOUD, n_win, out, st,
                               src, aux, n_win, n_t_or_pcap, dim, subsample, mode, normalise, th, L, p_max, n_points, out,
                               retry ? nullptr : armed_span(ctx, TDA_PROBE_RIPS_CLOUD), ctx->retry_ctr);
        },
        [&] {
            const RipsLayout L = total_layout(p_max, aux_bytes, CLOUD_NT);
            return launch_pass(ctx, rips_cloud_total_kernel<CLOUD_NT>, PASS_LAST, 0, CLOUD_NT, L.total, -1, n_win, out, st,
                               src, aux, n_win, n_t_or_pcap, dim, subsample, mode, normalise, th, L, p_max, n_points, out,
                               ctx->total_scratch, ctx->retry_ctr);
        });
}
```

Baseline: 4.830 million windows/s.

## Add compile-time fixed LDS layout EEG kernel for seven workgroups per CU

```diff
diff --git a/tda_eeg_audio_amd/csrc/corr_dist_dev.h b/tda_eeg_audio_amd/csrc/corr_dist_dev.h
--- a/tda_eeg_audio_amd/csrc/corr_dist_dev.h
+++ b/tda_eeg_audio_amd/csrc/corr_dist_dev.h
@@ -6,17 +6,18 @@
 #define CD_TSH 5
 #endif
 #define CD_MAXCH 64
+constexpr int cd_log2(int x) { return x <= 1 ? 0 : 1 + cd_log2(x >> 1); }
 
 typedef double d4 __attribute__((ext_vector_type(4)));
 
 
 
-template <int NPRE>
+template <int NPRE, int TCH = CD_TCH>
 __device__ __forceinline__ void cd_fetch(double (&pre)[NPRE], const double* __restrict__ X, int ld, int n_ch, int c0,
                                          int tc, int tid)
 {
-    constexpr int CPK = 256 / CD_TCH;
-    const int t = tid & (CD_TCH - 1), ch0 = tid >> CD_TSH;
+    constexpr int CPK = 256 / TCH, TSH = cd_log2(TCH);
+    const int t = tid & (TCH - 1), ch0 = tid >> TSH;
     const int toff = ch0 * ld + t;
     const bool live = t < tc;
 #pragma unroll
@@ -25,18 +26,19 @@
         pre[k] = (live && ch0 + CPK * k < n_ch) ? rowk[toff] : 0.0;
     }
 }
-template <int NPRE, int CSP>
+template <int NPRE, int CSP, int TCH = CD_TCH>
 __device__ __forceinline__ void cd_stash(const double (&pre)[NPRE], double* tile, const double* mean, int n_ch, int tc,
                                          int tid, bool centre)
 {
+    constexpr int TSH = cd_log2(TCH);
     double m[NPRE];
 #pragma unroll
-    for (int k = 0; k < NPRE; ++k) m[k] = centre ? mean[(tid + 256 * k) >> CD_TSH] : 0.0;
-    const int t = tid & (CD_TCH - 1);
+    for (int k = 0; k < NPRE; ++k) m[k] = centre ? mean[(tid + 256 * k) >> TSH] : 0.0;
+    const int t = tid & (TCH - 1);
     const bool live = t < tc;
 #pragma unroll
     for (int k = 0; k < NPRE; ++k) {
-        const int ch = (tid + 256 * k) >> CD_TSH;
+        const int ch = (tid + 256 * k) >> TSH;
         tile[t * CSP + ch] = live ? pre[k] - m[k] : 0.0;
     }
 }
@@ -44,12 +46,12 @@
 #define CD_RES_CHUNKS (256 / CD_TCH)
 
 
-template <int NB>
+template <int NB, int TCH = CD_TCH>
 struct CdLayout {
     static constexpr int CP = 16 * NB;
     static constexpr int CSP = CP + 1;
     static constexpr int NBLK = NB * (NB + 1) / 2;
-    static constexpr int TILE = CD_TCH * CSP;
+    static constexpr int TILE = TCH * CSP;
     static constexpr int ACCS = NBLK * 256;
     static constexpr size_t BYTES = sizeof(double) * ((size_t)TILE + ACCS + 2 * CP);
     __device__ static __forceinline__ int acc_index(int i, int j)
@@ -61,24 +63,26 @@
     }
 };
 
-template <int NB, bool RES>
+template <int NB, bool RES, int TCH = CD_TCH>
 __device__ __forceinline__ void cd_window_products(unsigned char* smem, const double* __restrict__ X, int n_ch, int n_t,
                                                    int ld)
 {
     constexpr int CP = 16 * NB;
     constexpr int CSP = CP + 1;
-    constexpr int NPRE = CP * CD_TCH / 256;
+    constexpr int NPRE = CP * TCH / 256;
     constexpr int NBLK = NB * (NB + 1) / 2;
     constexpr int MAXQ = (NBLK + 3) / 4;
     constexpr int NBUF = RES ? CD_RES_CHUNKS : 1;
+    static_assert(TCH == 16 || TCH == 32 || TCH == 64, "double trips of 16 samples");
+    static_assert(!RES || TCH == CD_TCH, "the resident variant keeps CD_RES_CHUNKS tiles of CD_TCH samples");
     double* tile = reinterpret_cast<double*>(smem);
-    double* accs = tile + CD_TCH * CSP;
+    double* accs = tile + TCH * CSP;
     double* mean = accs + NBLK * 256;
     double* sdev = mean + CP;
     const int tid = threadIdx.x, l = tid & 63, wv = uni(tid >> 6);
-    const int n_chunks = (n_t + CD_TCH - 1) / CD_TCH;
+    const int n_chunks = (n_t + TCH - 1) / TCH;
     double pre[NBUF][NPRE];
-    auto chunk_len = [&](int c) { const int r = n_t - c * CD_TCH; return r < CD_TCH ? r : CD_TCH; };
+    auto chunk_len = [&](int c) { const int r = n_t - c * TCH; return r < TCH ? r : TCH; };
     const double* lane_base = tile + (l >> 4) * CSP + (l & 15);
 
     d4 sacc = (d4){0.0, 0.0, 0.0, 0.0};
@@ -93,7 +97,7 @@
                 a[1][0] = p1[0]; a[1][1] = p1[4 * CSP];
                 sacc = __builtin_amdgcn_mfma_f64_16x16x4f64(a[0][0], 1.0, sacc, 0, 0, 0);
                 sacc = __builtin_amdgcn_mfma_f64_16x16x4f64(a[0][1], 1.0, sacc, 0, 0, 0);
-                const double* p2 = p0 + (16 * d + 16 < CD_TCH ? 16 * d + 16 : 0) * CSP;
+                const double* p2 = p0 + (16 * d + 16 < TCH ? 16 * d + 16 : 0) * CSP;
                 a[0][0] = p2[0]; a[0][1] = p2[4 * CSP];
                 sacc = __builtin_amdgcn_mfma_f64_16x16x4f64(a[1][0], 1.0, sacc, 0, 0, 0);
                 sacc = __builtin_amdgcn_mfma_f64_16x16x4f64(a[1][1], 1.0, sacc, 0, 0, 0);
@@ -103,22 +107,22 @@
     if constexpr (RES) {
 #pragma unroll
         for (int c = 0; c < NBUF; ++c)
-            if (c < n_chunks) cd_fetch<NPRE>(pre[c], X, ld, n_ch, c * CD_TCH, chunk_len(c), tid);
+            if (c < n_chunks) cd_fetch<NPRE, TCH>(pre[c], X, ld, n_ch, c * TCH, chunk_len(c), tid);
 #pragma unroll
         for (int c = 0; c < NBUF; ++c)
             if (c < n_chunks) {
-                cd_stash<NPRE, CSP>(pre[c], tile, mean, n_ch, chunk_len(c), tid, false);
+                cd_stash<NPRE, CSP, TCH>(pre[c], tile, mean, n_ch, chunk_len(c), tid, false);
                 __syncthreads();
                 sum_tile(chunk_len(c));
                 __syncthreads();
             }
     } else {
-        cd_fetch<NPRE>(pre[0], X, ld, n_ch, 0, chunk_len(0), tid);
+        cd_fetch<NPRE, TCH>(pre[0], X, ld, n_ch, 0, chunk_len(0), tid);
         for (int c = 0; c < n_chunks; ++c) {
-            cd_stash<NPRE, CSP>(pre[0], tile, mean, n_ch, chunk_len(c), tid, false);
+            cd_stash<NPRE, CSP, TCH>(pre[0], tile, mean, n_ch, chunk_len(c), tid, false);
             __syncthreads();
             const int c1 = (c + 1 < n_chunks) ? c + 1 : 0;
-            cd_fetch<NPRE>(pre[0], X, ld, n_ch, c1 * CD_TCH, chunk_len(c1), tid);
+            cd_fetch<NPRE, TCH>(pre[0], X, ld, n_ch, c1 * TCH, chunk_len(c1), tid);
             sum_tile(chunk_len(c));
             __syncthreads();
         }
@@ -173,7 +177,7 @@
         for (int d = 0; d < ntr; ++d) {
             load_ops(2 * d + 1, 1);
             run_ops(0);
-            load_ops(2 * d + 2 < CD_TCH / 8 ? 2 * d + 2 : 0, 0);
+            load_ops(2 * d + 2 < TCH / 8 ? 2 * d + 2 : 0, 0);
             run_ops(1);
         }
 #pragma unroll
@@ -187,16 +191,16 @@
 #pragma unroll
         for (int c = 0; c < NBUF; ++c)
             if (c < n_chunks) {
-                cd_stash<NPRE, CSP>(pre[c], tile, mean, n_ch, chunk_len(c), tid, true);
+                cd_stash<NPRE, CSP, TCH>(pre[c], tile, mean, n_ch, chunk_len(c), tid, true);
                 __syncthreads();
                 mfma_tile(c, chunk_len(c));
                 __syncthreads();
             }
     } else {
         for (int c = 0; c < n_chunks; ++c) {
-            cd_stash<NPRE, CSP>(pre[0], tile, mean, n_ch, chunk_len(c), tid, true);
-            __syncthreads();
-            if (c + 1 < n_chunks) cd_fetch<NPRE>(pre[0], X, ld, n_ch, (c + 1) * CD_TCH, chunk_len(c + 1), tid);
+            cd_stash<NPRE, CSP, TCH>(pre[0], tile, mean, n_ch, chunk_len(c), tid, true);
+            __syncthreads();
+            if (c + 1 < n_chunks) cd_fetch<NPRE, TCH>(pre[0], X, ld, n_ch, (c + 1) * TCH, chunk_len(c + 1), tid);
             mfma_tile(c, chunk_len(c));
             __syncthreads();
         }
diff --git a/tda_eeg_audio_amd/csrc/rips.hip b/tda_eeg_audio_amd/csrc/rips.hip
--- a/tda_eeg_audio_amd/csrc/rips.hip
+++ b/tda_eeg_audio_amd/csrc/rips.hip
@@ -547,21 +547,69 @@
 #define MISC_MIN (512 + 192)
 #define MISC_DONE (512 + 208)
 #define MISC_SORTCNT (512 + 224)
-#define MISC_SHARED (MISC_DONE + NT_MAX)
-#define MISC_CKEY (MISC_SHARED + 96)
-#define MISC_LIST MISC_CKEY
-#define MISC_LIST_BYTES (4 * NT_MAX + 1280)
-#define MISC_ADJ (MISC_LIST + MISC_LIST_BYTES)
-#define MISC_ADJC (MISC_ADJ + 128 * 16)
-#define MISC_BRANK (MISC_ADJC + 128 * 16)
-#define MISC_BYTES(ncls) (MISC_BRANK + 8 * (ncls))
-
-template <int NT, int NVW, int W, typename WT, bool NARROW, class KEYFN>
+template <int NTM, int NV>
+struct MiscT {
+    static constexpr int NVERT = NV;
+    static constexpr int AS = NV / 64;
+    static constexpr int SHARED = MISC_DONE + NTM;
+    static constexpr int CKEY = SHARED + 96;
+    static constexpr int LIST = CKEY;
+    static constexpr int LIST_BYTES = 4 * NTM + 1280;
+    static constexpr int ADJ = LIST + LIST_BYTES;
+    static constexpr int ADJC = ADJ + NV * AS * 8;
+    static constexpr int TL_BYTES = NV <= 64 ? 2 : 4;
+    static constexpr int BRANK = ADJC + NV * AS * 8;
+    static constexpr int bytes(int ncls) { return BRANK + 8 * ncls; }
+    static_assert(NV % 64 == 0 && LIST_BYTES >= 1024 + 16 * NV, "the labels of the Boruvka rounds lie in the list area");
+    static_assert(NTM * TL_BYTES <= NV * AS * 8, "the work list of phase d lives in adjc");
+    static_assert(NV <= 64 ? NTM <= 256 : true, "a two-byte code holds eight bits of thread index and six of vertex");
+};
+using ML = MiscT<NT_MAX, 128>;
+#define MISC_SHARED (ML::SHARED)
+#define MISC_CKEY (ML::CKEY)
+#define MISC_LIST (ML::LIST)
+#define MISC_LIST_BYTES (ML::LIST_BYTES)
+#define MISC_ADJ (ML::ADJ)
+#define MISC_ADJC (ML::ADJC)
+#define MISC_BRANK (ML::BRANK)
+#define MISC_BYTES(ncls) (ML::bytes(ncls))
+
+#define EEG_FIXED_NCH 48
+#define EEG_FIXED_TCH 16
+#define EEG_FIXED_LDS_MAX 23040
+struct RuntimeDmLayout {
+    static constexpr bool FIXED = false;
+    static constexpr int RANK = 0, ORD = 0, MEMBERS = 0, AUX = 0, MISC = 0;
+    using Misc = MiscT<NT_MAX, 128>;
+};
+template <int PB>
+struct EL {
+    static constexpr bool FIXED = true;
+    using Misc = MiscT<256, 64>;
+    static constexpr int E = EEG_FIXED_NCH * (EEG_FIXED_NCH - 1) / 2;
+    static constexpr int RANK = NL_A16(PB * E) + GUARD_BYTES;
+    static constexpr int ORD = NL_A16(RANK + 2 * E) + GUARD_BYTES;
+    static constexpr int MEMBERS = PB < 8 ? ORD : 4 * E;
+    static constexpr int AUX = NL_A16(ORD + 2 * E) + GUARD_BYTES;
+    static constexpr int MISC = NL_A16(AUX + 4 * E) + GUARD_BYTES;
+    static constexpr int MISC_NEED = Misc::bytes(8 * PB) > MISC_SORTCNT + 2 * 2048 ? Misc::bytes(8 * PB) : MISC_SORTCNT + 2 * 2048;
+    static constexpr int SWEEP = NL_A16(MISC + MISC_NEED) + GUARD_BYTES;
+    static constexpr int CD = (int)((CdLayout<3, EEG_FIXED_TCH>::BYTES + 15) & ~(size_t)15);
+    static constexpr int TOTAL = SWEEP > CD ? SWEEP : CD;
+    static_assert(TOTAL <= EEG_FIXED_LDS_MAX, "seven workgroups per CU: 18 LDS granules of 1,280 bytes each");
+    static_assert(EEG_FIXED_NCH <= Misc::NVERT && 4 * E + 512 <= 8 * CdLayout<3, EEG_FIXED_TCH>::TILE,
+                  "one vertex word; keys and row maxima fit the tile area in front of the accumulators");
+};
+
+template <int NT, int NVW, int W, typename WT, bool NARROW, class MLP = MiscT<NT_MAX, 128>, class KEYFN>
 __device__ __forceinline__ void rips_sweep(int n, int E, int Ev, const u16* rank, const u16* ord, Psi<W, WT>* psi, int psi_bytes,
                            unsigned char* misc, KEYFN keyfn, double* h0, int h0_cap, double* h1, int h1_cap,
                            int& out_k0, int& out_k1, int& out_status)
 {
     static_assert(!NARROW || W == 1, "the narrow layout is the point-cloud first pass");
+    using ML = MLP;
+    constexpr int AS = ML::AS, NV = ML::NVERT;
+    static_assert(NT <= (MISC_SHARED - MISC_DONE) && 64 * NVW <= NV, "the misc block covers this workgroup and its vertices");
     int psi_cap = 0;
     const int tid0 = threadIdx.x;
     const int lane0 = tid0 & 63, wave = uni(tid0 >> 6);
@@ -579,7 +627,7 @@
 
     if constexpr (!NARROW) for (int e = tid0; e < E; e += NT) psi[e] = pzero<W, WT>();
     for (int i = tid0; i < WB * W; i += NT) { brank[i] = -1; bkey[i] = 0.f; }
-    for (int i = tid0; i < 256; i += NT) { adj[i] = 0ull; adjc[i] = 0ull; }
+    for (int i = tid0; i < AS * NV; i += NT) { adj[i] = 0ull; adjc[i] = 0ull; }
     if (tid0 == 0) {
         u32* lc = reinterpret_cast<u32*>(misc + MISC_MIN);
         lc[0] = 0u; lc[1] = 0xffffffffu; lc[2] = 0u;
@@ -632,7 +680,7 @@
         for (int w = 0; w < NVW; ++w) { M[w] = 0; M0[w] = 0; Aj[w] = 0; Bj[w] = 0; }
         if (valid) {
 #pragma unroll
-            for (int w = 0; w < NVW; ++w) { Aj[w] = adj[2 * a + w]; Bj[w] = adj[2 * b + w]; M0[w] = Aj[w] & Bj[w]; }
+            for (int w = 0; w < NVW; ++w) { Aj[w] = adj[AS * a + w]; Bj[w] = adj[AS * b + w]; M0[w] = Aj[w] & Bj[w]; }
         }
         {
             volatile u32* turn = reinterpret_cast<volatile u32*>(misc + MISC_MIN) + 2;
@@ -648,9 +696,9 @@
             __builtin_amdgcn_fence(__ATOMIC_ACQUIRE, "workgroup");
             if (valid) {
 #pragma unroll
-                for (int w = 0; w < NVW; ++w) M[w] = (Aj[w] | adjc[2 * a + w]) & (Bj[w] | adjc[2 * b + w]);
-                atomicOr(reinterpret_cast<unsigned long long*>(&adjc[2 * a + (b >> 6)]), 1ull << (b & 63));
-                atomicOr(reinterpret_cast<unsigned long long*>(&adjc[2 * b + (a >> 6)]), 1ull << (a & 63));
+                for (int w = 0; w < NVW; ++w) M[w] = (Aj[w] | adjc[AS * a + w]) & (Bj[w] | adjc[AS * b + w]);
+                atomicOr(reinterpret_cast<unsigned long long*>(&adjc[AS * a + (b >> 6)]), 1ull << (b & 63));
+                atomicOr(reinterpret_cast<unsigned long long*>(&adjc[AS * b + (a >> 6)]), 1ull << (a & 63));
             }
             LDS_ORDER();
             if (lane == 0 && !(TDA_FAULT(1) && wave == 3)) *turn = (u32)wave + 1u;
@@ -659,7 +707,7 @@
             const int ta0 = tri2(a), tb0 = tri2(b);
 #pragma unroll
             for (int w = 0; w < NVW; ++w) {
-                u64 cc = (Aj[w] | adjc[2 * a + w]) & (Bj[w] | adjc[2 * b + w]) & ~M[w];
+                u64 cc = (Aj[w] | adjc[AS * a + w]) & (Bj[w] | adjc[AS * b + w]) & ~M[w];
                 while (cc) {
                     const int v0 = 64 * w + __builtin_ctzll(cc); cc &= cc - 1ull;
                     const bool ok1 = cc != 0ull; const int v1 = ok1 ? 64 * w + __builtin_ctzll(cc) : v0; cc &= cc - 1ull;
@@ -722,16 +770,17 @@
         const int lblA0 = compA, lblB0 = compB;
         int qpar = NT;
         if (par) {
+            constexpr int NH = NV / 64;
             int* bcomp = reinterpret_cast<int*>(misc + MISC_LIST + 1024);
-            u32* bbest2 = reinterpret_cast<u32*>(bcomp + 128);
-            int* bpar = reinterpret_cast<int*>(bcomp + 384);
+            u32* bbest2 = reinterpret_cast<u32*>(bcomp + NV);
+            int* bpar = reinterpret_cast<int*>(bcomp + 3 * NV);
             auto rounds = [&](int limit) {
-                if (wave == 0) { bcomp[lane] = lblA0; bcomp[64 + lane] = lblB0; }
-                if (tid < 256) bbest2[tid] = 0xffffffffu;
+                if (wave == 0) { bcomp[lane] = lblA0; if (NH == 2) bcomp[64 + lane] = lblB0; }
+                if (tid < 2 * NV) bbest2[tid] = 0xffffffffu;
                 __syncthreads();
                 bool live = is_cand && tid < limit, picked = false;
                 for (int round = 0; round < 64; ++round) {
-                    u32* bbest = bbest2 + 128 * (round & 1);
+                    u32* bbest = bbest2 + NV * (round & 1);
                     int ca = 0, cb2 = 0;
                     if (live) {
                         ca = bcomp[a]; cb2 = bcomp[b];
@@ -743,8 +792,9 @@
                     if (wave == 0) {
                         TDA_SOLO_BEGIN();
                         int pp[2];
-#pragma unroll
-                        for (int h = 0; h < 2; ++h) {
+                        pp[1] = 0;
+#pragma unroll
+                        for (int h = 0; h < NH; ++h) {
                             const int me = lane + 64 * h;
                             pp[h] = me;
                             const u32 bp = bbest[me];
@@ -755,18 +805,19 @@
                                 if (bbest[pp[h]] == bp && me < pp[h]) pp[h] = me;
                             }
                         }
-                        bpar[lane] = pp[0]; bpar[64 + lane] = pp[1];
+                        constexpr int HI = NH == 2 ? 64 : 0;
+                        bpar[lane] = pp[0]; if (NH == 2) bpar[64 + lane] = pp[1];
                         for (int it = 0; it < 8; ++it) {
-                            const int p0 = bpar[lane], p1 = bpar[64 + lane];
+                            const int p0 = bpar[lane], p1 = bpar[HI + lane];
                             const int g0 = bpar[p0], g1 = bpar[p1];
                             if (__ballot(g0 != p0 || g1 != p1) == 0ull) break;
-                            bpar[lane] = g0; bpar[64 + lane] = g1;
+                            bpar[lane] = g0; if (NH == 2) bpar[64 + lane] = g1;
                         }
-                        const int c0 = bcomp[lane], c1 = bcomp[64 + lane];
+                        const int c0 = bcomp[lane], c1 = bcomp[HI + lane];
                         const int n0 = bpar[c0], n1 = bpar[c1];
-                        bcomp[lane] = n0; bcomp[64 + lane] = n1;
-                        u32* other = bbest2 + 128 * ((round + 1) & 1);
-                        other[lane] = 0xffffffffu; other[64 + lane] = 0xffffffffu;
+                        bcomp[lane] = n0; if (NH == 2) bcomp[64 + lane] = n1;
+                        u32* other = bbest2 + NV * ((round + 1) & 1);
+                        other[lane] = 0xffffffffu; if (NH == 2) other[64 + lane] = 0xffffffffu;
                         TDA_SOLO_END();
                     }
                     __syncthreads();
@@ -791,7 +842,7 @@
                 __syncthreads();
                 rounds(qpar);
             }
-            if (wave == 0) { compA = bcomp[lane]; compB = bcomp[64 + lane]; }
+            if (wave == 0) { compA = bcomp[lane]; if (NH == 2) compB = bcomp[64 + lane]; }
         }
         if (wave == 0) {
             TDA_SOLO_BEGIN();
@@ -986,7 +1037,7 @@
                 if (NVW == 1 || vstar < 64) comp[0] = 1ull << vstar;
                 else comp[NVW - 1] = 1ull << (vstar - 64);
 #pragma unroll
-                for (int w = 0; w < NVW; ++w) { comp[w] |= adj[2 * vstar + w] & M[w]; rem[w] = M[w] & ~comp[w]; }
+                for (int w = 0; w < NVW; ++w) { comp[w] |= adj[AS * vstar + w] & M[w]; rem[w] = M[w] & ~comp[w]; }
                 bool changed = true;
                 while (changed) {
                     changed = false;
@@ -1005,7 +1056,7 @@
 #pragma unroll
                             for (int k = 0; k < 4; ++k)
 #pragma unroll
-                                for (int x = 0; x < NVW; ++x) nb[k][x] = adj[2 * u[k] + x];
+                                for (int x = 0; x < NVW; ++x) nb[k][x] = adj[AS * u[k] + x];
 #pragma unroll
                             for (int k = 0; k < 4; ++k) {
                                 u64 hit = 0ull;
@@ -1039,8 +1090,9 @@
         constexpr bool FTAB = WB * W * (int)sizeof(Psi<W, WT>) <= MISC_LIST_BYTES;
         constexpr int KMAX = FTAB ? 64 : LCAP;
         unsigned char* list = misc + MISC_LIST;
-        u32* tlist = reinterpret_cast<u32*>(adjc);
-        static_assert(4 * NT <= 128 * 16 && NT / 64 <= 8, "the work list lives in adjc; nine words per sum");
+        using TL = std::conditional_t<ML::TL_BYTES == 2, u16, u32>;
+        TL* tlist = reinterpret_cast<TL*>(adjc);
+        static_assert((int)sizeof(TL) * NT <= NV * AS * 8 && NT / 64 <= 8, "the work list lives in adjc; nine words per sum");
         const bool cum_lane = lane == 8 || (lane < 8 && lane > wave);
         const int ntri = __builtin_popcount(m0) + __builtin_popcount(m1) + __builtin_popcount(m2) + __builtin_popcount(m3);
         int tstart, ttot;
@@ -1086,7 +1138,7 @@
                     while (left[wi] != 0ull && (u32)(nxt - t0) < (u32)NT) {
                         const int v = 64 * wi + __builtin_ctzll(left[wi]);
                         left[wi] &= left[wi] - 1ull;
-                        tlist[nxt - t0] = ((u32)tid << 8) | (u32)v;
+                        tlist[nxt - t0] = (TL)(((u32)tid << 8) | (u32)v);
                         ++nxt;
                     }
                 }
@@ -1098,7 +1150,7 @@
                 if (t0 + (wave << 6) < ttot) {
                     const bool item = t0 + tid < ttot;
                     if (item) {
-                        code = tlist[tid];
+                        code = (u32)tlist[tid];
                         const int op = (int)(code >> 8), v = (int)(code & 255u);
                         const u32 pk = ord[r0 + op];
                         const int oa = (int)(pk >> 8), ob = (int)(pk & 255u);
@@ -1411,10 +1463,10 @@
         }
         }
         if (valid && tid < clen) {
-            atomicOr(reinterpret_cast<unsigned long long*>(&adj[2 * a + (b >> 6)]), 1ull << (b & 63));
-            atomicOr(reinterpret_cast<unsigned long long*>(&adj[2 * b + (a >> 6)]), 1ull << (a & 63));
-        }
-        if (tid < 256) adjc[tid] = 0ull;
+            atomicOr(reinterpret_cast<unsigned long long*>(&adj[AS * a + (b >> 6)]), 1ull << (b & 63));
+            atomicOr(reinterpret_cast<unsigned long long*>(&adj[AS * b + (a >> 6)]), 1ull << (a & 63));
+        }
+        if (tid < AS * NV) adjc[tid] = 0ull;
         if (tid == 0) {
             lcnt[0] = 0u; lcnt[1] = 0xffffffffu; lcnt[2] = 0u; shared->cov_min[0] = 0x7fffffff;
             if (lcnt[3]) shared->status = TDA_WIN_NOT_CONVERGED;
@@ -1436,8 +1488,8 @@
                 while (rr < Ev) {
                     const u32 pk = ord[rr];
                     const int ea = (int)(pk >> 8), eb = (int)(pk & 255u);
-                    u64 common = adj[2 * ea] & adj[2 * eb];
-                    if (NVW == 2) common |= adj[2 * ea + 1] & adj[2 * eb + 1];
+                    u64 common = adj[AS * ea] & adj[AS * eb];
+                    if (NVW == 2) common |= adj[AS * ea + 1] & adj[AS * eb + 1];
                     if (common == 0ull) { covered = false; break; }
                     rr += NT;
                 }
@@ -1453,8 +1505,8 @@
                 for (int r2 = from + tid; r2 < ru; r2 += NT) {
                     const u32 pk = ord[r2];
                     const int ea = (int)(pk >> 8), eb = (int)(pk & 255u);
-                    atomicOr(reinterpret_cast<unsigned long long*>(&adj[2 * ea + (eb >> 6)]), 1ull << (eb & 63));
-                    atomicOr(reinterpret_cast<unsigned long long*>(&adj[2 * eb + (ea >> 6)]), 1ull << (ea & 63));
+                    atomicOr(reinterpret_cast<unsigned long long*>(&adj[AS * ea + (eb >> 6)]), 1ull << (eb & 63));
+                    atomicOr(reinterpret_cast<unsigned long long*>(&adj[AS * eb + (ea >> 6)]), 1ull << (ea & 63));
                 }
                 PROF_COUNT(35, ru - from);
                 from = ru;
@@ -1647,19 +1699,20 @@
     __device__ __forceinline__ float operator()(int r, int, int) const { return sortable_f32(skey[r]); }
 };
 
-template <int NT, int NVW, int W, typename WT, bool TOTAL = false>
+template <int NT, int NVW, int W, typename WT, bool TOTAL = false, class LP = RuntimeDmLayout>
 __device__ __forceinline__ void rips_dm_rest(unsigned char* smem, const int win, int n, float thresh, const u32* vmax, u32 kmin_thread,
                              const RipsLayout& L, const RipsOut& out, u64* psi_g = nullptr)
 {
+    static_assert(!LP::FIXED || (!TOTAL && NVW == 1 && NT == 256), "the fixed layout is a first pass on one vertex word");
     const int tid = threadIdx.x;
     const int E = tri2(n);
     u32* key32 = reinterpret_cast<u32*>(smem);
-    u16* members = reinterpret_cast<u16*>(smem + L.off_members);
+    u16* members = reinterpret_cast<u16*>(smem + (LP::FIXED ? LP::MEMBERS : L.off_members));
     Psi<W, WT>* psi = reinterpret_cast<Psi<W, WT>*>(smem);
-    u16* rank = reinterpret_cast<u16*>(smem + L.off_rank);
-    u16* ord = reinterpret_cast<u16*>(smem + L.off_ord);
-    u32* skey = reinterpret_cast<u32*>(smem + L.off_aux);
-    unsigned char* misc = smem + L.off_misc;
+    u16* rank = reinterpret_cast<u16*>(smem + (LP::FIXED ? LP::RANK : L.off_rank));
+    u16* ord = reinterpret_cast<u16*>(smem + (LP::FIXED ? LP::ORD : L.off_ord));
+    u32* skey = reinterpret_cast<u32*>(smem + (LP::FIXED ? LP::AUX : L.off_aux));
+    unsigned char* misc = smem + (LP::FIXED ? LP::MISC : L.off_misc);
     u32* red = reinterpret_cast<u32*>(misc + MISC_MIN);
     u32* cursor = reinterpret_cast<u32*>(misc + MISC_SORTCNT);
     int* wsum = reinterpret_cast<int*>(misc + MISC_WV);
@@ -1679,7 +1732,7 @@
                              out.h0 + (size_t)win * out.h0_cap * 2, out.h0_cap,
                              out.h1 + (size_t)win * out.h1_cap * 2, out.h1_cap, k0, k1, st);
     else
-    rips_sweep<NT, NVW, W, WT, false>(n, E, Ev, rank, ord, psi, 0, misc, kf,
+    rips_sweep<NT, NVW, W, WT, false, typename LP::Misc>(n, E, Ev, rank, ord, psi, 0, misc, kf,
                        out.h0 + (size_t)win * out.h0_cap * 2, out.h0_cap,
                        out.h1 + (size_t)win * out.h1_cap * 2, out.h1_cap, k0, k1, st);
     st |= guard_check(smem, L);
@@ -2023,7 +2076,7 @@
     __device__ __forceinline__ int ld_of(int w) const { return (int)ld[w]; }
 };
 
-template <int NB, bool RES, int W, typename WT, bool TOTAL = false, class SRC>
+template <int NB, bool RES, int W, typename WT, bool TOTAL = false, class LP = RuntimeDmLayout, class SRC>
 __device__ __forceinline__ void eeg_one_window(unsigned char* smem, const SRC& src, int w, int n_ch,
                                                int n_t, float thresh, const RipsLayout& L, const RipsOut& out,
                                                double* __restrict__ dist, double* __restrict__ corr,
@@ -2031,9 +2084,10 @@
 {
     const int tid = threadIdx.x, l = tid & 63, wv = tid >> 6;
     PROF_BEGIN();
-    cd_window_products<NB, RES>(smem, src.at(w), n_ch, n_t, src.ld_of(w));
-    const double* accs = reinterpret_cast<const double*>(smem) + CdLayout<NB>::TILE;
-    const double* sdev = accs + CdLayout<NB>::ACCS + CdLayout<NB>::CP;
+    constexpr int TCH = LP::FIXED ? EEG_FIXED_TCH : CD_TCH;
+    cd_window_products<NB, RES, TCH>(smem, src.at(w), n_ch, n_t, src.ld_of(w));
+    const double* accs = reinterpret_cast<const double*>(smem) + CdLayout<NB, TCH>::TILE;
+    const double* sdev = accs + CdLayout<NB, TCH>::ACCS + CdLayout<NB, TCH>::CP;
     const double fact = 1.0 / (double)(n_t - 1);
     auto dist_at = [&](int i, int j, double* r_out) {
         double r = (accs[CdLayout<NB>::acc_index(i, j)] * fact / sdev[i]) / sdev[j];
@@ -2072,7 +2126,7 @@
     }
     __syncthreads();
     PROF_MARK(0);
-    rips_dm_rest<256, TOTAL ? 2 : 1, W, WT, TOTAL>(smem, w, n_ch, thresh, vmax, kmin_thread, L, out, psi_g);
+    rips_dm_rest<256, TOTAL ? 2 : 1, W, WT, TOTAL, LP>(smem, w, n_ch, thresh, vmax, kmin_thread, L, out, psi_g);
 }
 
 #ifndef TDA_EEG_WIDE_WAVES
@@ -2112,6 +2166,18 @@
             eeg_one_window<NB, RES, W, WT>(smem, windows, win, n_ch, n_t, thresh, L, out, dist, corr);
         RETRY_SCAN_END()
     }
+}
+#ifndef TDA_EEG_FIXED_WAVES
+#define TDA_EEG_FIXED_WAVES 7
+#endif
+template <class SRC, typename WT>
+__global__ void __launch_bounds__(256, TDA_EEG_FIXED_WAVES)
+eeg_window_fixed_kernel(SRC windows, int n_win, int n_ch, int n_t, float thresh, RipsLayout L, RipsOut out,
+                        double* __restrict__ dist, double* __restrict__ corr, unsigned long long* __restrict__ retry_ctr)
+{
+    extern __shared__ __attribute__((aligned(16))) unsigned char smem[];
+    if ((int)blockIdx.x < n_win)
+        eeg_one_window<3, false, 1, WT, false, EL<(int)sizeof(WT)>>(smem, windows, (int)blockIdx.x, n_ch, n_t, thresh, L, out, dist, corr);
 }
 template <int NB, bool RES, class SRC>
 __global__ void __launch_bounds__(256, 2)
@@ -2217,6 +2283,23 @@
     L.guard[0] = NL::PSI; L.guard[1] = NL::MISC; L.guard[2] = NL::AUX; L.guard[3] = NL::TOTAL; L.guard[4] = NL::TOTAL;
     L.n_guard = 4;
     return L;
+}
+
+template <int PB>
+static RipsLayout make_eeg_fixed_layout(int n_ch)
+{
+    using F = EL<PB>;
+    RipsLayout L;
+    L.off_members = F::MEMBERS; L.off_rank = F::RANK; L.off_ord = F::ORD; L.off_aux = F::AUX; L.off_misc = F::MISC;
+    L.off_psi = 0; L.psi_bytes = 0; L.off_cursor = F::MISC + MISC_SORTCNT; L.off_rscr = F::MISC;
+    L.total = n_ch <= EEG_FIXED_NCH ? F::TOTAL : 0;
+    L.guard[0] = F::RANK; L.guard[1] = F::ORD; L.guard[2] = F::AUX; L.guard[3] = F::MISC; L.guard[4] = F::SWEEP;
+    L.n_guard = 5;
+    return L;
+}
+extern "C" __attribute__((visibility("default"))) int tda_eeg_fixed_lds_bytes(int bits)
+{
+    return bits == 32 ? EL<4>::TOTAL : bits == 64 ? EL<8>::TOTAL : 0;
 }
 
 static tda_status order_h1(tda_ctx* ctx, double* h1, int h1_cap, int* h1_cnt, int n_win, hipStream_t st)
@@ -2315,8 +2398,9 @@
 }
 
 template <bool RES, class SRC>
-static auto eeg_kernel(const SRC* src, int bits, bool retry)
-{
+static auto eeg_kernel(const SRC* src, int bits, bool retry, bool fixed)
+{
+    if (fixed) return bits == 32 ? eeg_window_fixed_kernel<SRC, u32> : eeg_window_fixed_kernel<SRC, u64>;
     switch (bits) {
     case 32: return eeg_kernel_of<3, RES, 1, false, u32>(src);
     case 64: return retry ? eeg_kernel_of<3, RES, 1, true, u64>(src) : eeg_kernel_of<3, RES, 1, false, u64>(src);
@@ -2331,13 +2415,16 @@
 {
     const int aux = n_ch * (n_ch - 1) / 2 * 4;
     const int cd_bytes = (int)((CdLayout<3>::BYTES + 15) & ~(size_t)15);
+    static const bool runtime_first = getenv("TDA_EEG_RUNTIME_FIRST") != nullptr;
     return run_ladder(ctx, rips_ladder::eeg_rungs(ctx->words_dm), n_win, out, st,
         [&](int bits, bool retry) -> tda_status {
-            RipsLayout L = make_layout(n_ch, bits / 8, aux, 256);
-            if ((size_t)L.total < CdLayout<3>::BYTES) L.total = cd_bytes;
+            const RipsLayout F = bits == 32 ? make_eeg_fixed_layout<4>(n_ch) : make_eeg_fixed_layout<8>(n_ch);
+            const bool fixed = !RES && !retry && !runtime_first && (bits == 32 || bits == 64) && F.total != 0;
+            RipsLayout L = fixed ? F : make_layout(n_ch, bits / 8, aux, 256);
+            if (!fixed && (size_t)L.total < CdLayout<3>::BYTES) L.total = cd_bytes;
             if (L.total > LDS_MAX) TDA_FAIL(ctx, TDA_ERR_UNSUPPORTED, "window too large for LDS");
             const int rgrid = (bits >> 6) >= 8 ? RETRY_GRID_WIDE : RETRY_GRID;
-            return launch_pass(ctx, eeg_kernel<RES>(&win, bits, retry), retry ? PASS_RETRY : PASS_FIRST, rgrid, 256, L.total,
+            return launch_pass(ctx, eeg_kernel<RES>(&win, bits, retry, fixed), retry ? PASS_RETRY : PASS_FIRST, rgrid, 256, L.total,
                                TDA_PROBE_RIPS_DM, n_win, out, st, win, n_win, n_ch, n_t, th, L, out, dist, corr, ctx->retry_ctr);
         },
         [&] {
```

Result: no change. 4.793 million windows/s (-0.8%).
